# jalberse/shimmer

Hardware: AMD Instinct MI355X
Metric: Mray/s (primary+secondary) at 1024^2 256spp Ganesha; 1/2/4/8-GPU scaling (higher is better)
Workload: dtype f32

## Files before the change

### include/shimmer_hip.h

```cpp
#ifndef SHIMMER_HIP_H
#define SHIMMER_HIP_H

#include <stdint.h>

#ifdef __cplusplus
extern "C" {
#endif

#define SHM_ABI_VERSION 10

#if defined(__GNUC__)
#define SHM_API __attribute__((visibility("default")))
#else
#define SHM_API
#endif

typedef enum ShmError {
    SHM_OK = 0,
    SHM_ERR_INVALID_ARGUMENT = -1,
    SHM_ERR_UNSUPPORTED = -2,
    SHM_ERR_DEVICE = -3,
    SHM_ERR_NO_DEVICE = -4,
    SHM_ERR_OUT_OF_MEMORY = -5,
    SHM_ERR_INTERNAL = -6
// ... 358 lines not shown
    double ms_gather;
    uint64_t gather_bytes;
} ShmStats;

typedef struct ShmRay {
    float o[3];
    float d[3];
    float t_max;
    float pad;
} ShmRay;

typedef struct ShmHit {
    int32_t prim;
    float t;
    float b0, b1, b2;
    float phi;
    uint32_t instance;
    uint32_t pad;
} ShmHit;

typedef struct ShmScene ShmScene;

SHM_API int shm_scene_create(const ShmSceneDesc* desc, int device, ShmScene** out);
SHM_API void shm_scene_destroy(ShmScene* scene);

SHM_API int shm_scene_shading_records(ShmScene* scene, uint64_t* n_records_out, double* build_ms_out);

SHM_API int shm_film_clear(ShmScene* scene);
SHM_API int shm_render_wave(ShmScene* scene, const ShmRenderParams* params, const ShmTile* tiles, uint32_t n_tiles,
                    int32_t sample_begin, int32_t sample_end, ShmStats* stats);
SHM_API int shm_film_read(ShmScene* scene, ShmFilmPixel* film_out);
SHM_API int shm_film_device_ptr(ShmScene* scene, void** ptr_out, uint64_t* bytes_out);

SHM_API int shm_render_device(ShmScene* scene, const ShmRenderParams* params, const ShmTile* tiles, uint32_t n_tiles,
                              ShmStats* stats);
SHM_API int shm_render(ShmScene* scene, const ShmRenderParams* params, const ShmTile* tiles, uint32_t n_tiles,
               ShmFilmPixel* film, ShmStats* stats);

SHM_API int shm_trace_closest(ShmScene* scene, const ShmRay* rays, uint32_t n, ShmHit* hits_out, ShmStats* stats);
SHM_API int shm_trace_any(ShmScene* scene, const ShmRay* rays, uint32_t n, uint8_t* occluded_out, ShmStats* stats);
SHM_API int shm_trace_closest_device(ShmScene* scene, const void* rays_dev, uint32_t n, void* hits_dev, int repeat,
                             ShmStats* stats);
SHM_API int shm_trace_any_device(ShmScene* scene, const void* rays_dev, uint32_t n, void* occluded_dev, int repeat,
                         ShmStats* stats);


SHM_API int shm_shard_tiles(uint32_t n_tiles, uint32_t tiles_per_row, int32_t rank, int32_t world, int32_t rows_per_block,
                            uint32_t* idx_out, uint32_t* n_out);

#define SHM_DIST_ID_BYTES 128
SHM_API int shm_dist_unique_id(uint8_t id_out[SHM_DIST_ID_BYTES]);
SHM_API int shm_dist_init(ShmScene* scene, int32_t rank, int32_t world, const uint8_t id[SHM_DIST_ID_BYTES]);
SHM_API int shm_dist_finalize(ShmScene* scene);
SHM_API int shm_render_sharded(ShmScene* scene, const ShmRenderParams* params, ShmStats* stats);
enum { SHM_REDUCE_SUM = 0, SHM_REDUCE_MAX = 1, SHM_REDUCE_MIN = 2 };
SHM_API int shm_dist_barrier(ShmScene* scene);
SHM_API int shm_dist_allreduce_f64(ShmScene* scene, double* values , uint32_t n , int32_t op );
SHM_API int shm_dist_allgather_f64(ShmScene* scene, const double* mine, uint32_t n, double* all_out );
typedef struct ShmDistInfo {
    int32_t rank, world;
    int32_t rccl_ranks;
    int32_t rccl_device;
    int32_t rccl_version;
    int32_t hip_runtime_version;
    int32_t rows_per_block;
    uint32_t n_my_tiles;
    char librccl_path[256];
    char libamdhip_path[256];
} ShmDistInfo;
SHM_API int shm_dist_info(ShmScene* scene, ShmDistInfo* out);
SHM_API int shm_device_synchronize(int32_t device);
SHM_API int shm_dist_selftest(ShmScene* scene);

SHM_API int shm_render_multi(const ShmSceneDesc* desc, const int32_t* devices, int32_t n_devices, const ShmRenderParams* params,
                             ShmFilmPixel* film_out, ShmStats* stats_per_device);

SHM_API const char* shm_last_error(void);
SHM_API int shm_device_count(void);


SHM_API int shm_bvh_build(const float* prim_bounds, uint32_t n, int split_method, ShmBvhNode* nodes_out,
                  uint32_t* n_nodes_out, uint32_t* prim_order_out);
SHM_API int shm_bounds3_probe(const float a[6], const float b[6], const float p[3], float out[16]);
SHM_API int shm_tile_bounds(const int32_t pixel_bounds[4], int32_t tile_w, int32_t tile_h, ShmTile* tiles_out,
                    uint32_t* n_out);
SHM_API int shm_camera_perspective(const float world_from_camera[16], float fov_deg, const int32_t full_resolution[2],
                           float lens_radius, float focal_distance, ShmCamera* out,
                           float render_from_world_out[16]);
SHM_API int shm_camera_orthographic(const float world_from_camera[16], const int32_t full_resolution[2], float lens_radius,
                            float focal_distance, ShmCamera* out, float render_from_world_out[16]);
enum { SHM_RENDER_SPACE_CAMERA_WORLD = 0, SHM_RENDER_SPACE_CAMERA = 1, SHM_RENDER_SPACE_WORLD = 2 };
typedef struct ShmCameraParams {
    uint32_t kind;
    uint32_t render_space;
    float world_from_camera[16];
    float fov_deg;
    int32_t full_resolution[2];
    float lens_radius, focal_distance;
    float frame_aspect_ratio;
    uint32_t has_screen_window;
    float screen_window[4];
} ShmCameraParams;
SHM_API int shm_camera_create(const ShmCameraParams* params, ShmCamera* out, float render_from_world_out[16]);
SHM_API int shm_camera_spherical(const float world_from_camera[16], uint32_t mapping, const int32_t full_resolution[2], uint32_t render_space, ShmCamera* out,
                                 float render_from_world_out[16]);
SHM_API int shm_integrator_render(const char* name, const ShmSceneDesc* scene, int device, int32_t max_depth, int regularize,
                          int sample_lights, int sample_bsdf, int32_t samples_per_pixel, int32_t seed, int disable_pixel_jitter,
                          int disable_wavelength_jitter, ShmFilmPixel* film_out, ShmStats* stats_out, int32_t* n_waves_out);
SHM_API int shm_film_get_image(const ShmFilmPixel* film, uint64_t n_pixels, const float output_rgb_from_sensor_rgb[9], int write_fp16,
                       float* rgb_out);
SHM_API int shm_write_pfm(const char* path, const float* rgb, int32_t width, int32_t height);
typedef struct ShmPlyMesh {
    uint32_t n_vertices, n_tri_indices, n_quad_indices, n_face_indices;
    float* p;
    float* n;
    float* uv;
    int32_t* tri_indices;
    int32_t* quad_indices;
    int32_t* face_indices;
} ShmPlyMesh;
SHM_API int shm_ply_read(const char* filename, ShmPlyMesh* out);
SHM_API void shm_ply_free(ShmPlyMesh* mesh);

typedef struct ShmPbrtScene {
    ShmSceneDesc desc;
    ShmRenderParams params;
    char integrator[32];
    char output_filename[256];
    void* owner;
    float output_rgb_from_sensor_rgb[9];
} ShmPbrtScene;
SHM_API int shm_scene_load_pbrt(const char* path, ShmPbrtScene** out);
SHM_API int shm_scene_parse_pbrt(const char* text, const char* base_dir, ShmPbrtScene** out);
SHM_API void shm_pbrt_free(ShmPbrtScene* scene);
SHM_API int shm_pbrt_tokenize(const char* text, char* out, uint64_t capacity, uint32_t* n_tokens);
SHM_API int shm_pbrt_parse_params(const char* text, char* out_json, uint64_t capacity);
SHM_API int shm_blackbody_dense(float temperature_kelvin, float out471[471]);
SHM_API int shm_look_at(const float eye[3], const float look[3], const float up[3], float world_from_camera_out[16]);
typedef struct ShmLoadedImage {
    uint32_t n_levels, n_channels, file_channels, has_color_space;
    uint64_t n_texel_floats;
    ShmImageLevel* levels;
    float* texels;
} ShmLoadedImage;
SHM_API int shm_image_load_png(const char* path, const char* encoding, uint32_t wrap , int build_pyramid, ShmLoadedImage* out);
SHM_API void shm_image_free(ShmLoadedImage* image);

#ifdef __cplusplus
}
#endif
#endif
```

### shimmer_amd/abi.py

```python
import ctypes as C
import os
from pathlib import Path

ROOT = Path(__file__).resolve().parent
LIB_PATH = ROOT / "csrc" / "libshimmer_hip.so"

SHM_ABI_VERSION = 10
SHM_OK = 0
SHM_DIST_ID_BYTES = 128
SHM_SHAPE_TRIANGLE, SHM_SHAPE_SPHERE, SHM_SHAPE_BILINEAR_PATCH, SHM_SHAPE_INSTANCE = 0, 1, 2, 3
SHM_SPECTRUM_CONSTANT, SHM_SPECTRUM_DENSE, SHM_SPECTRUM_PIECEWISE_LINEAR = 0, 1, 2
SHM_SPECTRUM_RGB_ALBEDO, SHM_SPECTRUM_RGB_UNBOUNDED, SHM_SPECTRUM_RGB_ILLUMINANT = 3, 4, 5
SHM_MATERIAL_DIFFUSE, SHM_MATERIAL_CONDUCTOR, SHM_MATERIAL_DIELECTRIC, SHM_MATERIAL_THIN_DIELECTRIC = 0, 1, 2, 3
SHM_MATERIAL_COATED_DIFFUSE, SHM_MATERIAL_COATED_CONDUCTOR, SHM_MATERIAL_MIX = 4, 5, 6
SHM_MATERIAL_DIFFUSE_TRANSMISSION = 8
SHM_LIGHT_POINT, SHM_LIGHT_DIFFUSE_AREA, SHM_LIGHT_UNIFORM_INFINITE, SHM_LIGHT_IMAGE_INFINITE = 0, 1, 2, 3
SHM_LIGHT_DISTANT, SHM_LIGHT_SPOT = 4, 5
SHM_SPECTRUM_IMAGE_TEXTURE, SHM_SPECTRUM_TEXTURE_NODE = 6, 7
SHM_SPECTEX_LEAF, SHM_SPECTEX_SCALED, SHM_SPECTEX_MIX, SHM_SPECTEX_DIRECTION_MIX = 0, 1, 2, 3
SHM_TEXMAP_UV, SHM_TEXMAP_SPHERICAL, SHM_TEXMAP_CYLINDRICAL, SHM_TEXMAP_PLANAR = 0, 1, 2, 3
SHM_TEXMAP_POINT3D = 4
SHM_TEXFILTER_POINT, SHM_TEXFILTER_BILINEAR, SHM_TEXFILTER_TRILINEAR, SHM_TEXFILTER_EWA = 0, 1, 2, 3
SHM_FILTER_BOX, SHM_FILTER_GAUSSIAN, SHM_FILTER_MITCHELL, SHM_FILTER_SINC, SHM_FILTER_TRIANGLE = 0, 1, 2, 3, 4
SHM_WRAP_BLACK, SHM_WRAP_CLAMP, SHM_WRAP_REPEAT, SHM_WRAP_OCTAHEDRAL_SPHERE = 0, 1, 2, 3
# ... 144 lines not shown

class ShmRenderParams(C.Structure):
    _fields_ = [("seed", C.c_uint64), ("samples_per_pixel", C.c_int32), ("max_depth", C.c_int32), ("regularize", C.c_uint8),
                ("disable_pixel_jitter", C.c_uint8), ("disable_wavelength_jitter", C.c_uint8), ("force_diffuse", C.c_uint8),
                ("integrator", C.c_uint8), ("sample_lights", C.c_uint8), ("sample_bsdf", C.c_uint8), ("disable_texture_filtering", C.c_uint8),
                ("disable_reference_quirks", C.c_uint8), ("sampler", C.c_uint8), ("sampler_randomization", C.c_uint8), ("pad", C.c_uint8 * 5)]


class ShmTile(C.Structure):
    _fields_ = [("x0", C.c_int32), ("y0", C.c_int32), ("x1", C.c_int32), ("y1", C.c_int32)]


class ShmFilmPixel(C.Structure):
    _fields_ = [("rgb_sum", C.c_double * 3), ("weight_sum", C.c_double)]


class ShmStats(C.Structure):
    _fields_ = [("paths", C.c_uint64), ("rays_closest", C.c_uint64), ("rays_any", C.c_uint64), ("nodes_closest", C.c_uint64),
                ("tris_closest", C.c_uint64), ("nodes_any", C.c_uint64), ("tris_any", C.c_uint64), ("ms_total", C.c_double),
                ("ms_trace_closest", C.c_double), ("ms_trace_any", C.c_double), ("ms_shade", C.c_double),
                ("launches_closest", C.c_uint32), ("launches_any", C.c_uint32), ("ms_gather", C.c_double), ("gather_bytes", C.c_uint64)]

    def as_dict(self):
        return {name: getattr(self, name) for name, _ in self._fields_}


class ShmRay(C.Structure):
    _fields_ = [("o", C.c_float * 3), ("d", C.c_float * 3), ("t_max", C.c_float), ("pad", C.c_float)]


class ShmHit(C.Structure):
    _fields_ = [("prim", C.c_int32), ("t", C.c_float), ("b0", C.c_float), ("b1", C.c_float), ("b2", C.c_float),
                ("phi", C.c_float), ("instance", C.c_uint32), ("pad", C.c_uint32)]


assert C.sizeof(ShmMaterial) == 64 + 4 * 32 + 48 and C.sizeof(ShmFloatTexture) == 48 and C.sizeof(ShmBvhNode) == 32 and C.sizeof(ShmRay) == 32 and C.sizeof(ShmHit) == 32 and C.sizeof(ShmFilmPixel) == 32

class ShmPbrtScene(C.Structure):
    _fields_ = [("desc", ShmSceneDesc), ("params", ShmRenderParams), ("integrator", C.c_char * 32), ("output_filename", C.c_char * 256), ("owner", C.c_void_p),
                ("output_rgb_from_sensor_rgb", C.c_float * 9)]


class ShmCameraParams(C.Structure):
    _fields_ = [("kind", C.c_uint32), ("render_space", C.c_uint32), ("world_from_camera", C.c_float * 16), ("fov_deg", C.c_float),
                ("full_resolution", C.c_int32 * 2), ("lens_radius", C.c_float), ("focal_distance", C.c_float), ("frame_aspect_ratio", C.c_float),
                ("has_screen_window", C.c_uint32), ("screen_window", C.c_float * 4)]


class ShmLoadedImage(C.Structure):
    _fields_ = [("n_levels", C.c_uint32), ("n_channels", C.c_uint32), ("file_channels", C.c_uint32), ("has_color_space", C.c_uint32),
                ("n_texel_floats", C.c_uint64), ("levels", C.POINTER(ShmImageLevel)), ("texels", c_float_p)]


class ShmDistInfo(C.Structure):
    _fields_ = [("rank", C.c_int32), ("world", C.c_int32), ("rccl_ranks", C.c_int32), ("rccl_device", C.c_int32), ("rccl_version", C.c_int32),
                ("hip_runtime_version", C.c_int32), ("rows_per_block", C.c_int32), ("n_my_tiles", C.c_uint32), ("librccl_path", C.c_char * 256),
                ("libamdhip_path", C.c_char * 256)]

    def as_dict(self):
        return {n: (getattr(self, n).decode() if n.endswith("_path") else getattr(self, n)) for n, _ in self._fields_}


SHM_REDUCE_SUM, SHM_REDUCE_MAX, SHM_REDUCE_MIN = 0, 1, 2

EXPORTS = {
    "shm_scene_create": (C.c_int, [C.POINTER(ShmSceneDesc), C.c_int, C.POINTER(C.c_void_p)]),
    "shm_scene_destroy": (None, [C.c_void_p]),
    "shm_film_clear": (C.c_int, [C.c_void_p]),
    "shm_scene_shading_records": (C.c_int, [C.c_void_p, C.POINTER(C.c_uint64), C.POINTER(C.c_double)]),
    "shm_render_wave": (C.c_int, [C.c_void_p, C.POINTER(ShmRenderParams), C.POINTER(ShmTile), C.c_uint32, C.c_int32, C.c_int32,
                                  C.POINTER(ShmStats)]),
    "shm_film_read": (C.c_int, [C.c_void_p, C.c_void_p]),
    "shm_film_device_ptr": (C.c_int, [C.c_void_p, C.POINTER(C.c_void_p), C.POINTER(C.c_uint64)]),
    "shm_render_device": (C.c_int, [C.c_void_p, C.POINTER(ShmRenderParams), C.POINTER(ShmTile), C.c_uint32, C.POINTER(ShmStats)]),
    "shm_render": (C.c_int, [C.c_void_p, C.POINTER(ShmRenderParams), C.POINTER(ShmTile), C.c_uint32, C.c_void_p, C.POINTER(ShmStats)]),
    "shm_trace_closest": (C.c_int, [C.c_void_p, C.c_void_p, C.c_uint32, C.c_void_p, C.POINTER(ShmStats)]),
    "shm_trace_any": (C.c_int, [C.c_void_p, C.c_void_p, C.c_uint32, C.c_void_p, C.POINTER(ShmStats)]),
    "shm_trace_closest_device": (C.c_int, [C.c_void_p, C.c_void_p, C.c_uint32, C.c_void_p, C.c_int, C.POINTER(ShmStats)]),
    "shm_trace_any_device": (C.c_int, [C.c_void_p, C.c_void_p, C.c_uint32, C.c_void_p, C.c_int, C.POINTER(ShmStats)]),
    "shm_last_error": (C.c_char_p, []),
    "shm_device_count": (C.c_int, []),
    "shm_bvh_build": (C.c_int, [c_float_p, C.c_uint32, C.c_int, C.POINTER(ShmBvhNode), c_u32_p, c_u32_p]),
    "shm_bounds3_probe": (C.c_int, [c_float_p, c_float_p, c_float_p, c_float_p]),
    "shm_tile_bounds": (C.c_int, [C.POINTER(C.c_int32), C.c_int32, C.c_int32, C.POINTER(ShmTile), c_u32_p]),
    "shm_camera_perspective": (C.c_int, [c_float_p, C.c_float, C.POINTER(C.c_int32), C.c_float, C.c_float, C.POINTER(ShmCamera), c_float_p]),
    "shm_integrator_render": (C.c_int, [C.c_char_p, C.POINTER(ShmSceneDesc), C.c_int, C.c_int32, C.c_int, C.c_int, C.c_int, C.c_int32, C.c_int32, C.c_int, C.c_int,
                                        C.c_void_p, C.POINTER(ShmStats), C.POINTER(C.c_int32)]),
    "shm_camera_orthographic": (C.c_int, [c_float_p, C.POINTER(C.c_int32), C.c_float, C.c_float, C.POINTER(ShmCamera), c_float_p]),
    "shm_film_get_image": (C.c_int, [C.c_void_p, C.c_uint64, c_float_p, C.c_int, c_float_p]),
    "shm_write_pfm": (C.c_int, [C.c_char_p, c_float_p, C.c_int32, C.c_int32]),
    "shm_ply_read": (C.c_int, [C.c_char_p, C.c_void_p]),
    "shm_ply_free": (None, [C.c_void_p]),
    "shm_shard_tiles": (C.c_int, [C.c_uint32, C.c_uint32, C.c_int32, C.c_int32, C.c_int32, c_u32_p, c_u32_p]),
    "shm_dist_unique_id": (C.c_int, [C.c_void_p]),
    "shm_dist_init": (C.c_int, [C.c_void_p, C.c_int32, C.c_int32, C.c_void_p]),
    "shm_dist_finalize": (C.c_int, [C.c_void_p]),
    "shm_render_sharded": (C.c_int, [C.c_void_p, C.POINTER(ShmRenderParams), C.POINTER(ShmStats)]),
    "shm_dist_selftest": (C.c_int, [C.c_void_p]),
    "shm_dist_barrier": (C.c_int, [C.c_void_p]),
    "shm_dist_allreduce_f64": (C.c_int, [C.c_void_p, C.POINTER(C.c_double), C.c_uint32, C.c_int32]),
    "shm_dist_allgather_f64": (C.c_int, [C.c_void_p, C.POINTER(C.c_double), C.c_uint32, C.POINTER(C.c_double)]),
    "shm_dist_info": (C.c_int, [C.c_void_p, C.POINTER(ShmDistInfo)]),
    "shm_device_synchronize": (C.c_int, [C.c_int32]),
    "shm_scene_load_pbrt": (C.c_int, [C.c_char_p, C.POINTER(C.POINTER(ShmPbrtScene))]),
    "shm_scene_parse_pbrt": (C.c_int, [C.c_char_p, C.c_char_p, C.POINTER(C.POINTER(ShmPbrtScene))]),
    "shm_pbrt_free": (None, [C.POINTER(ShmPbrtScene)]),
    "shm_pbrt_tokenize": (C.c_int, [C.c_char_p, C.c_char_p, C.c_uint64, c_u32_p]),
    "shm_pbrt_parse_params": (C.c_int, [C.c_char_p, C.c_char_p, C.c_uint64]),
    "shm_blackbody_dense": (C.c_int, [C.c_float, c_float_p]),
    "shm_look_at": (C.c_int, [c_float_p, c_float_p, c_float_p, c_float_p]),
    "shm_image_load_png": (C.c_int, [C.c_char_p, C.c_char_p, C.c_uint32, C.c_int, C.POINTER(ShmLoadedImage)]),
    "shm_image_free": (None, [C.POINTER(ShmLoadedImage)]),
    "shm_camera_create": (C.c_int, [C.POINTER(ShmCameraParams), C.POINTER(ShmCamera), c_float_p]),
    "shm_camera_spherical": (C.c_int, [c_float_p, C.c_uint32, C.POINTER(C.c_int32), C.c_uint32, C.POINTER(ShmCamera), c_float_p]),
    "shm_render_multi": (C.c_int, [C.POINTER(ShmSceneDesc), C.POINTER(C.c_int32), C.c_int32, C.POINTER(ShmRenderParams), C.c_void_p, C.POINTER(ShmStats)]),
}

_lib = None


class ShimmerHipError(RuntimeError):
    pass


def load_library(path=None):
    global _lib
    if _lib is not None and path is None:
        return _lib
    if path is None and os.environ.get("SHM_LIB"):
        path = os.environ["SHM_LIB"]
    p = Path(path) if path else LIB_PATH
    if not p.exists():
        raise ShimmerHipError(f"{p} not found: run `python -c 'import __graft_entry__ as g; g.build()'` "
                              "(hipcc --offload-arch=gfx950). There is no CPU fallback for the render path.")
    lib = C.CDLL(str(p), mode=getattr(os, "RTLD_NOW", 2))
    host_only = os.environ.get("SHM_HOST_ONLY") == "1"
    for name, (res, args) in EXPORTS.items():
        if host_only and not hasattr(lib, name):
            continue
        fn = getattr(lib, name)
        fn.restype = res
        fn.argtypes = args
    if path is None:
        _lib = lib
    return lib


PROBE_LIB_PATH = LIB_PATH.parent / "libshimmer_hip_probe.so"
_probe = None


def load_probe_library():
    global _probe
    if _probe is None:
        if not PROBE_LIB_PATH.exists():
            raise ShimmerHipError(f"{PROBE_LIB_PATH} not found: run `python -c 'import __graft_entry__ as g; g.build()'`")
        lib = C.CDLL(str(PROBE_LIB_PATH), mode=getattr(os, "RTLD_NOW", 2))
        lib.shm_debug_eval_leaf.restype = C.c_int
        lib.shm_debug_eval_leaf.argtypes = [C.c_int, C.c_int, c_u32_p, C.c_uint32, c_u32_p, C.c_uint32, C.POINTER(C.c_int)]
        lib.shm_probe_last_error.restype = C.c_char_p
        _probe = lib
    return _probe


def check(lib, rc, what):
    if rc != SHM_OK:
# ... 3 lines not shown
```

### shimmer_amd/csrc/host/flatten.h

```cpp
#pragma once
#include <stdio.h>
#include <stdlib.h>

#include <algorithm>
#include <cmath>
#include <string>
#include <utility>
#include <vector>

#include "../shm/filter.h"
#include "../shm/scene.h"

static_assert(sizeof(ShmMaterial) == 240 && sizeof(ShmFloatTexture) == 48 && sizeof(ShmSpectrumTexture) == 64 && sizeof(ShmSpectrum) == 32 && sizeof(ShmBvhNode) == 32 && sizeof(ShmPrimitive) == 16,
              "POD layouts of include/shimmer_hip.h (mirrored by shimmer_amd/abi.py)");
namespace shm_host {

struct FlatScene {
    std::vector<ShmBvhNode> nodes;
    std::vector<shm::PrimRec> prim_recs;
    std::vector<ShmPrimitive> primitives;
    std::vector<uint32_t> mesh_flags;
    std::vector<uint32_t> vi;
    std::vector<float> vn, vs, vuv;
    std::vector<ShmSphere> spheres;
    std::vector<shm::PatchExtra> patches;
    std::vector<uint32_t> patch_vi;
    std::vector<float> patch_vn, patch_vuv;
    std::vector<ShmMaterial> materials;
    std::vector<ShmLight> lights;
    std::vector<shm::PrimRec> light_prim_recs;
    bool has_diffuse_transmission = false;
    bool has_directed_lights = false;
    std::vector<uint32_t> infinite_lights;
    std::vector<float> spectrum_data;
    std::vector<float> sensor_r, sensor_g, sensor_b;
    ShmCamera camera;
    ShmFilm film;
    uint32_t max_leaf_depth = 0;
    float scene_radius = 0.0f;
    uint64_t n_quadric_patch_prims = 0;
    bool has_spheres = false;
    bool has_layered = false;
    bool has_rough_dielectric = false;
    bool has_class[4] = {false, false, false, false};
    bool diffuse_only = true;
    std::vector<ShmImageTexture> image_textures;
    std::vector<ShmImageLevel> image_levels;
    std::vector<float> texel_data;
    std::vector<float> rgb2spec_scale, rgb2spec_data, cs_illuminant, ewa_lut;
    uint32_t rgb2spec_res = 0;
    bool has_textures = false;
    bool has_material_textures = false, has_image_light = false;
    double area_plain_diffuse = 0.0, area_total = 0.0;
    uint64_t n_plain_diffuse_prims = 0;
    std::vector<ShmInstance> instances;
    bool has_instances = false;
    std::vector<ShmFloatTexture> float_textures;
    std::vector<shm::FloatTexRange> ftex_ranges;
    std::vector<shm::FloatTexOp> ftex_ops;
    std::vector<ShmSpectrumTexture> spectrum_textures;
    std::vector<shm::FloatTexRange> stex_ranges;
    std::vector<shm::FloatTexOp> stex_ops;
    std::vector<shm::ImageLightRec> image_lights;
    std::vector<float> dist_data;

    shm::SceneView view() const {
        shm::SceneView v;
        v.quirks_off = 0;
        v.zsobol = 0;
        v.call_copy = nullptr;
        v.inst_roots = nullptr;
        v.tri_shade = nullptr;
        v.nodes = nodes.data();
        v.n_nodes = (uint32_t)nodes.size();
        v.prim_recs = prim_recs.data();
        v.primitives = primitives.data();
        v.n_primitives = (uint32_t)primitives.size();
        v.mesh_flags = mesh_flags.data();
        v.vi = vi.data();
        v.vn = vn.data();
        v.vs = vs.data();
        v.vuv = vuv.data();
        v.spheres = spheres.data();
        v.patches = patches.data();
        v.patch_vi = patch_vi.data();
        v.patch_vn = patch_vn.data();
        v.patch_vuv = patch_vuv.data();
        v.materials = materials.data();
        v.lights = lights.data();
        v.n_lights = (uint32_t)lights.size();
        v.light_prim_recs = light_prim_recs.empty() ? nullptr : light_prim_recs.data();
        v.infinite_lights = infinite_lights.data();
        v.n_infinite_lights = (uint32_t)infinite_lights.size();
        v.spectrum_data = spectrum_data.data();
        v.scene_radius = scene_radius;
        v.camera = camera;
        for (int i = 0; i < 4; ++i) v.pixel_bounds[i] = film.pixel_bounds[i];
        v.filter_radius[0] = film.filter_radius[0];
        v.filter_radius[1] = film.filter_radius[1];
        v.filter_kind = film.filter;
        v.imaging_ratio = film.imaging_ratio;
        v.max_component_value = film.max_component_value;
        v.sensor_r_bar = sensor_r.data();
        v.sensor_g_bar = sensor_g.data();
        v.sensor_b_bar = sensor_b.data();
        v.image_textures = image_textures.data();
        v.image_levels = image_levels.data();
        v.texel_data = texel_data.data();
        v.rgb2spec_res = rgb2spec_res;
        v.rgb2spec_scale = rgb2spec_scale.data();
        v.rgb2spec_data = rgb2spec_data.data();
        v.cs_illuminant = cs_illuminant.data();
        v.ewa_lut = ewa_lut.data();
        v.instances = instances.data();
        v.float_textures = float_textures.data();
        v.ftex_ranges = ftex_ranges.data();
        v.ftex_ops = ftex_ops.data();
        v.spectrum_textures = spectrum_textures.data();
        v.stex_ranges = stex_ranges.data();
        v.stex_ops = stex_ops.data();
        v.image_lights = image_lights.data();
        v.dist_data = dist_data.data();
        return v;
    }
};

inline bool check_spectrum(const ShmSpectrum& s, uint32_t n_floats, std::string& err, uint32_t n_textures = 0, bool* is_texture = nullptr) {
    if (s.kind == SHM_SPECTRUM_TEXTURE_NODE) {
        if (!is_texture) { err = "a spectrum texture is not valid in this slot"; return false; }
        *is_texture = true;
        return true;
    }
    if (s.kind == SHM_SPECTRUM_IMAGE_TEXTURE) {
        if (s.offset >= n_textures) { err = n_textures ? "image texture index out of range" : "an image texture is not valid in this slot"; return false; }
        if (is_texture) *is_texture = true;
        return true;
    }
    if (s.kind == SHM_SPECTRUM_CONSTANT || s.kind == SHM_SPECTRUM_RGB_ALBEDO || s.kind == SHM_SPECTRUM_RGB_UNBOUNDED) return true;
    if (s.kind == SHM_SPECTRUM_DENSE || s.kind == SHM_SPECTRUM_RGB_ILLUMINANT) {
        if ((uint64_t)s.offset + s.n > n_floats) { err = "dense spectrum out of range"; return false; }
        return true;
    }
    if (s.kind == SHM_SPECTRUM_PIECEWISE_LINEAR) {
        if (s.n < 2 || (uint64_t)s.offset + 2ull * s.n > n_floats) { err = "piecewise spectrum out of range"; return false; }
        return true;
    }
    err = "unknown spectrum kind";
    return false;
}

inline float build_pc1d(const float* f, size_t n, std::vector<float>& pool, size_t func_off, size_t cdf_off) {
    for (size_t i = 0; i < n; ++i) pool[func_off + i] = f[i] < 0.0f ? -f[i] : f[i];
    pool[cdf_off] = 0.0f;
    for (size_t i = 1; i <= n; ++i) pool[cdf_off + i] = pool[cdf_off + i - 1] + pool[func_off + i - 1] * (1.0f - 0.0f) / (float)n;
    const float func_int = pool[cdf_off + n];
// ... 485 lines not shown
    out.light_prim_recs.assign(out.lights.size(), shm::PrimRec{});
    for (uint32_t i = 0; i < out.lights.size(); ++i)
        if (out.lights[i].kind == SHM_LIGHT_DIFFUSE_AREA) out.light_prim_recs[i] = out.prim_recs[out.lights[i].primitive];
    for (uint32_t i = 0; i < out.lights.size(); ++i) {
        if (out.lights[i].kind != SHM_LIGHT_SPOT) continue;
        const ShmSpotLight& sp = d->spot_lights[out.lights[i].primitive];
        shm::PrimRec& r = out.light_prim_recs[i];
        for (int k = 0; k < 3; ++k) { r.p0[k] = sp.light_from_render[k]; r.p1[k] = sp.light_from_render[4 + k]; r.p2[k] = sp.light_from_render[8 + k]; }
        r.mesh = shm::float_to_bits(sp.cos_falloff_start);
        r.tri = shm::float_to_bits(sp.cos_falloff_end);
    }

    if (d->n_instances) out.instances.assign(d->instances, d->instances + d->n_instances);
    {
        struct Item { uint32_t node, depth; bool inner; };
        std::vector<Item> st;
        st.push_back({0u, 0u, false});
        uint64_t visited = 0;
        const uint64_t visit_cap = (uint64_t)d->n_nodes * (1ull + d->n_instances);
        while (!st.empty()) {
            auto [i, depth, inner] = st.back();
            st.pop_back();
            if (i >= d->n_nodes) { err = "BVH child index out of range"; return SHM_ERR_INVALID_ARGUMENT; }
            if (++visited > visit_cap) { err = "BVH is not a tree"; return SHM_ERR_INVALID_ARGUMENT; }
            const ShmBvhNode& n = d->nodes[i];
            if (n.n_prims > 0) {
                if ((uint64_t)n.offset + n.n_prims > d->n_primitives) { err = "BVH leaf range out of bounds"; return SHM_ERR_INVALID_ARGUMENT; }
                if (depth > out.max_leaf_depth) out.max_leaf_depth = depth;
                for (uint32_t k = 0; k < n.n_prims; ++k) {
                    const ShmPrimitive& pr = out.primitives[n.offset + k];
                    if (pr.shape_kind != SHM_SHAPE_INSTANCE) {
                        if (inner && pr.area_light >= 0) { err = "an instanced primitive cannot carry an area light"; return SHM_ERR_UNSUPPORTED; }
                        continue;
                    }
                    if (inner) { err = "an instanced primitive cannot itself be an instance"; return SHM_ERR_UNSUPPORTED; }
                    if (n.n_prims != 1) { err = "an instance must be alone in its BVH leaf"; return SHM_ERR_UNSUPPORTED; }
                    const ShmInstance& in = out.instances[pr.shape_index];
                    if (in.root_node == 0 || in.root_node >= d->n_nodes) { err = "instance root node out of range"; return SHM_ERR_INVALID_ARGUMENT; }
                    st.push_back({in.root_node, depth + 2, true});
                }
            } else {
                if (n.axis > 2) { err = "BVH axis out of range"; return SHM_ERR_INVALID_ARGUMENT; }
                if (n.offset <= i) { err = "BVH second child must follow its parent"; return SHM_ERR_INVALID_ARGUMENT; }
                st.push_back({n.offset, depth + 1, inner});
                st.push_back({i + 1, depth + 1, inner});
            }
        }
    }
    if (getenv("SHM_DEBUG")) fprintf(stderr, "[shm] flatten: %u nodes, %u prims, max leaf depth %u\n", d->n_nodes, d->n_primitives, out.max_leaf_depth);
    if (out.max_leaf_depth >= 64) { err = "BVH deeper than the reference's 64-entry traversal stack"; return SHM_ERR_UNSUPPORTED; }
    for (ShmMaterial& m : out.materials) {
        if (m.kind == SHM_MATERIAL_DIFFUSE_TRANSMISSION) {
            ShmSpectrum zero;
            memset(&zero, 0, sizeof(zero));
            zero.kind = SHM_SPECTRUM_CONSTANT;
            m.c = m.d = zero;
            m.conductor_from_reflectance = 0;
            for (int k = 1; k < 8; ++k) m.float_tex[k] = 0u;
        }
        const bool tex_a = m.a.kind == SHM_SPECTRUM_IMAGE_TEXTURE || m.a.kind == SHM_SPECTRUM_TEXTURE_NODE;
        bool any_float_tex = false;
        for (int k = 0; k < 8; ++k) any_float_tex = any_float_tex || m.float_tex[k] != 0u;
        m.pad[0] = (m.kind == SHM_MATERIAL_DIFFUSE && !tex_a && !any_float_tex && m.normal_map == 0u) ? 1u : 0u;
    }
    for (const shm::PrimRec& pr : out.prim_recs) {
        const bool plain = pr.material < out.materials.size() && (out.materials[pr.material].pad[0] & 1u);
        if (plain) out.n_plain_diffuse_prims += 1u;
        double area = 0.0;
        if (pr.kind_index & shm::PRIM_SPHERE_BIT) { const double r = d->spheres[pr.kind_index & shm::PRIM_INDEX_MASK].radius; area = 4.0 * 3.14159265358979 * r * r; }
        else if (pr.kind_index & shm::PRIM_PATCH_BIT) area = out.patches[pr.kind_index & shm::PRIM_INDEX_MASK].area;
        else if (!(pr.kind_index & shm::PRIM_INSTANCE_BIT)) {
            const double ax = (double)pr.p1[0] - pr.p0[0], ay = (double)pr.p1[1] - pr.p0[1], az = (double)pr.p1[2] - pr.p0[2];
            const double bx = (double)pr.p2[0] - pr.p0[0], by = (double)pr.p2[1] - pr.p0[1], bz = (double)pr.p2[2] - pr.p0[2];
            const double cx = ay * bz - az * by, cy = az * bx - ax * bz, cz = ax * by - ay * bx;
            area = 0.5 * std::sqrt(cx * cx + cy * cy + cz * cz);
        }
        if (area == area && area < 1e300) { out.area_total += area; if (plain) out.area_plain_diffuse += area; }
    }
    out.has_material_textures = out.has_textures;
    out.has_textures = out.has_material_textures || out.has_image_light;
    return SHM_OK;
}

}
```

### shimmer_amd/csrc/host/host_mirror.cpp

```cpp
#include <stdio.h>
#include <string.h>

#include <algorithm>
#include <atomic>
#include <cmath>
#include <new>
#include <stdexcept>
#include <string>
#include <thread>
#include <vector>

#include "../../../include/shimmer_hip.h"
#include "../shm/path.h"

extern "C" __attribute__((visibility("hidden"))) void shm_set_last_error(const char* msg);

namespace {

struct B3 {
    float mn[3], mx[3];
};
inline B3 b3_default() {
    B3 b;
    for (int i = 0; i < 3; ++i) { b.mn[i] = 3.40282346638528859812e+38f; b.mx[i] = -3.40282346638528859812e+38f; }
    return b;
}
inline float fmin_rs(float a, float b) { return (b != b) ? a : ((a != a) ? b : (a < b ? a : b)); }
inline float fmax_rs(float a, float b) { return (b != b) ? a : ((a != a) ? b : (a > b ? a : b)); }
inline B3 b3_union(const B3& a, const B3& b) {
    B3 r;
    for (int i = 0; i < 3; ++i) { r.mn[i] = fmin_rs(a.mn[i], b.mn[i]); r.mx[i] = fmax_rs(a.mx[i], b.mx[i]); }
    return r;
}
inline B3 b3_union_point(const B3& a, const float p[3]) {
    B3 r;
    for (int i = 0; i < 3; ++i) { r.mn[i] = fmin_rs(a.mn[i], p[i]); r.mx[i] = fmax_rs(a.mx[i], p[i]); }
    return r;
}
inline float b3_surface_area(const B3& b) {
    float dx = b.mx[0] - b.mn[0], dy = b.mx[1] - b.mn[1], dz = b.mx[2] - b.mn[2];
    return 2.0f * (dx * dy + dx * dz + dy * dz);
}
inline int b3_max_dimension(const B3& b) {
    float dx = b.mx[0] - b.mn[0], dy = b.mx[1] - b.mn[1], dz = b.mx[2] - b.mn[2];
    if (dx > dy && dx > dz) return 0;
    return (dy > dz) ? 1 : 2;
}

struct BvhPrimitive {
    uint32_t primitive_index;
    B3 bounds;
    float centroid(int dim) const {
        return 0.5f * bounds.mn[dim] + bounds.mx[dim] * 0.5f;
    }
};

struct BuildNode {
    B3 bounds;
    int left = -1, right = -1;
    uint8_t split_axis = 0;
    uint32_t first_prim_offset = 0;
    uint32_t n_primitives = 0;
};

struct BuildTask {
    size_t begin, end;
    int top_index;
    std::vector<BuildNode> nodes;
};
constexpr uint32_t TASK_PLACEHOLDER = 0xffffffffu;

struct Builder {
    BvhPrimitive* prims;
    std::vector<BuildNode> build_nodes;
    uint32_t* ordered;
    int split_method;
    std::vector<BuildTask>* tasks = nullptr;
    size_t grain = 0;

    template <typename Pred>
    static size_t partition(BvhPrimitive* a, size_t n, Pred pred) {
        size_t split_index = 0;
        size_t front = 0, back = n;
        while (front < back) {
            if (!pred(a[front])) {
                bool swapped = false;
                while (back > front + 1) {
                    --back;
                    if (pred(a[back])) {
                        std::swap(a[front], a[back]);
                        swapped = true;
                        break;
                    }
                }
                if (!swapped) break;
            }
// ... 65 lines not shown
            return mid;
        };
        if (split_method == 0) {
            float pmid = (cb.mn[dim] + cb.mx[dim]) / 2.0f;
            split_index = partition(prims + begin, n, [dim, pmid](const BvhPrimitive& p) { return p.centroid(dim) < pmid; });
            if (split_index == 0 || split_index == n) split_index = median_split();
        } else {
            split_index = median_split();
        }
        int left = build(begin, begin + split_index);
        int right = build(begin + split_index, end);
        BuildNode& node = build_nodes[node_idx];
        node.bounds = b3_union(build_nodes[left].bounds, build_nodes[right].bounds);
        node.left = left;
        node.right = right;
        node.split_axis = (uint8_t)dim;
        return node_idx;
    }
};

thread_local std::string g_host_err;

struct M4 {
    double m[4][4];
};
M4 m4_identity() {
    M4 r;
    for (int i = 0; i < 4; ++i) for (int j = 0; j < 4; ++j) r.m[i][j] = (i == j) ? 1.0 : 0.0;
    return r;
}
M4 m4_mul(const M4& a, const M4& b) {
    M4 r;
    for (int i = 0; i < 4; ++i)
        for (int j = 0; j < 4; ++j) {
            double s = 0;
            for (int k = 0; k < 4; ++k) s += a.m[i][k] * b.m[k][j];
            r.m[i][j] = s;
        }
    return r;
}
bool m4_inverse(const M4& a, M4& out) {
    double aug[4][8];
    for (int i = 0; i < 4; ++i)
        for (int j = 0; j < 4; ++j) { aug[i][j] = a.m[i][j]; aug[i][j + 4] = (i == j) ? 1.0 : 0.0; }
    for (int c = 0; c < 4; ++c) {
        int piv = c;
        for (int r = c + 1; r < 4; ++r) if (std::fabs(aug[r][c]) > std::fabs(aug[piv][c])) piv = r;
        if (aug[piv][c] == 0.0) return false;
        if (piv != c) for (int j = 0; j < 8; ++j) std::swap(aug[c][j], aug[piv][j]);
        double inv = 1.0 / aug[c][c];
        for (int j = 0; j < 8; ++j) aug[c][j] *= inv;
        for (int r = 0; r < 4; ++r) {
            if (r == c) continue;
            double f = aug[r][c];
            if (f != 0.0) for (int j = 0; j < 8; ++j) aug[r][j] -= f * aug[c][j];
        }
    }
    for (int i = 0; i < 4; ++i) for (int j = 0; j < 4; ++j) out.m[i][j] = aug[i][j + 4];
    return true;
}
M4 m4_scale(double x, double y, double z) { M4 r = m4_identity(); r.m[0][0] = x; r.m[1][1] = y; r.m[2][2] = z; return r; }
M4 m4_translate(double x, double y, double z) { M4 r = m4_identity(); r.m[0][3] = x; r.m[1][3] = y; r.m[2][3] = z; return r; }
void m4_to_f32(const M4& a, float* out) { for (int i = 0; i < 4; ++i) for (int j = 0; j < 4; ++j) out[i * 4 + j] = (float)a.m[i][j]; }
void m4_point(const M4& a, const double p[3], double out[3]) {
    double r[4];
    for (int i = 0; i < 4; ++i) r[i] = a.m[i][0] * p[0] + a.m[i][1] * p[1] + a.m[i][2] * p[2] + a.m[i][3];
    for (int i = 0; i < 3; ++i) out[i] = (r[3] == 1.0) ? r[i] : r[i] / r[3];
}

}

extern "C" {

int shm_bounds3_probe(const float a[6], const float b[6], const float p[3], float out[16]) {
    if (!a || !b || !p || !out) return SHM_ERR_INVALID_ARGUMENT;
    B3 ba, bb;
    for (int k = 0; k < 3; ++k) { ba.mn[k] = a[k]; ba.mx[k] = a[3 + k]; bb.mn[k] = b[k]; bb.mx[k] = b[3 + k]; }
    const B3 u = b3_union(ba, bb), up = b3_union_point(ba, p);
    for (int k = 0; k < 3; ++k) { out[k] = u.mn[k]; out[3 + k] = u.mx[k]; out[6 + k] = up.mn[k]; out[9 + k] = up.mx[k]; }
    out[12] = b3_surface_area(ba);
    out[13] = (ba.mx[0] - ba.mn[0]) * (ba.mx[1] - ba.mn[1]) * (ba.mx[2] - ba.mn[2]);
    out[14] = (float)b3_max_dimension(ba);
    out[15] = 0.0f;
    return SHM_OK;
}

int shm_bvh_build(const float* prim_bounds, uint32_t n, int split_method, ShmBvhNode* nodes_out,
                  uint32_t* n_nodes_out, uint32_t* prim_order_out) {
    if (!prim_bounds || n == 0 || !nodes_out || !n_nodes_out || !prim_order_out || split_method < 0 || split_method > 1)
        return SHM_ERR_INVALID_ARGUMENT;
    std::vector<BvhPrimitive> prims(n);
    for (uint32_t i = 0; i < n; ++i) {
        prims[i].primitive_index = i;
        for (int k = 0; k < 3; ++k) {
            prims[i].bounds.mn[k] = prim_bounds[6ull * i + k];
            prims[i].bounds.mx[k] = prim_bounds[6ull * i + 3 + k];
            if (prim_bounds[6ull * i + k] != prim_bounds[6ull * i + k]) return SHM_ERR_INVALID_ARGUMENT;
        }
    }
    unsigned n_threads = std::min(std::max(std::thread::hardware_concurrency(), 1u), 64u);
    if (const char* e = getenv("SHM_BVH_THREADS")) { const int v = atoi(e); if (v >= 1 && v <= 1024) n_threads = (unsigned)v; }
    if (n < 65536u) n_threads = 1;
    std::vector<BuildTask> tasks;
    Builder b;
    b.prims = prims.data();
    b.build_nodes.reserve(n_threads > 1 ? 1024 : 2ull * n);
    b.ordered = prim_order_out;
    b.split_method = split_method;
    if (n_threads > 1) { b.tasks = &tasks; b.grain = n / 64u; b.fold_threads = std::min(n_threads, 16u); }
    b.build(0, n);
    if (!tasks.empty()) {
        std::atomic<size_t> next{0};
        auto worker = [&]() {
            for (size_t t = next.fetch_add(1); t < tasks.size(); t = next.fetch_add(1)) {
                Builder sub;
                sub.prims = prims.data();
                sub.ordered = prim_order_out;
                sub.split_method = split_method;
                sub.build_nodes.reserve(2 * (tasks[t].end - tasks[t].begin));
                sub.build(tasks[t].begin, tasks[t].end);
                tasks[t].nodes.swap(sub.build_nodes);
            }
        };
        std::vector<std::thread> pool;
        try {
            for (unsigned t = 1; t < std::min<size_t>(n_threads, tasks.size()); ++t) pool.emplace_back(worker);
        } catch (...) {}
        worker();
        for (std::thread& t : pool) t.join();
        auto bounds_of = [&](int i) -> const B3& { const BuildNode& c = b.build_nodes[i]; return c.n_primitives == TASK_PLACEHOLDER ? tasks[c.first_prim_offset].nodes[0].bounds : c.bounds; };
        for (size_t i = b.build_nodes.size(); i-- > 0;) {
            BuildNode& node = b.build_nodes[i];
            if (node.n_primitives == 0) node.bounds = b3_union(bounds_of(node.left), bounds_of(node.right));
        }
    }
    std::vector<uint32_t> final_index(b.build_nodes.size());
    uint64_t total64 = 0;
    for (size_t i = 0; i < b.build_nodes.size(); ++i) {
        final_index[i] = (uint32_t)total64;
        total64 += b.build_nodes[i].n_primitives == TASK_PLACEHOLDER ? tasks[b.build_nodes[i].first_prim_offset].nodes.size() : 1u;
    }
    if (total64 > 0xffffffffull) return SHM_ERR_UNSUPPORTED;
    const uint32_t total = (uint32_t)total64;
    std::atomic<int> rc_emit{SHM_OK};
    std::atomic<uint64_t> n_in_leaves{0};
    auto emit = [&](const BuildNode& bn, uint32_t base, ShmBvhNode& ln, uint64_t& leaf_prims) {
        memset(&ln, 0, sizeof(ln));
        for (int k = 0; k < 3; ++k) { ln.bmin[k] = bn.bounds.mn[k]; ln.bmax[k] = bn.bounds.mx[k]; }
        if (bn.n_primitives > 0) {
            if (bn.n_primitives >= 65536) rc_emit = SHM_ERR_UNSUPPORTED;
            ln.offset = bn.first_prim_offset;
            ln.n_prims = (uint16_t)bn.n_primitives;
            ln.axis = 0;
            leaf_prims += bn.n_primitives;
        } else {
            ln.offset = base;
            ln.n_prims = 0;
            ln.axis = bn.split_axis;
        }
    };
    {
        uint64_t leaf_prims = 0;
        for (size_t i = 0; i < b.build_nodes.size(); ++i) {
            const BuildNode& bn = b.build_nodes[i];
            if (bn.n_primitives == TASK_PLACEHOLDER) continue;
            emit(bn, bn.n_primitives == 0 ? final_index[bn.right] : 0u, nodes_out[final_index[i]], leaf_prims);
// ... 407 lines not shown
```

### shimmer_amd/csrc/render.hip

```cpp
#include <chrono>
#include "wavefront.h"
#include "host/integrator.hpp"

std::string& shm_err() {
    thread_local std::string e;
    return e;
}
#define g_err shm_err()

namespace {

__global__ void k_expand_tiles(const ShmTile* tiles, const uint32_t* tile_offset, uint32_t n_tiles, uint32_t* pixels) {
    uint32_t t = blockIdx.x * blockDim.x + threadIdx.x;
    if (t >= n_tiles) return;
    ShmTile tl = tiles[t];
    uint32_t k = tile_offset[t];
    for (int x = tl.x0; x < tl.x1; ++x)
        for (int y = tl.y0; y < tl.y1; ++y) pixels[k++] = (uint32_t)x | ((uint32_t)y << 16);
}

#include "k_generate.inl"

__global__ void __launch_bounds__(256) k_build_tri_shade(SceneView sv, PrimRec* prim_recs, TriShadeRec* recs, uint32_t n_prims, uint32_t* n_built, uint32_t plain_only) {
    const uint32_t i = blockIdx.x * blockDim.x + threadIdx.x;
// ... 148 lines not shown
};
struct FilterKernels {
    FilteredGenerateKernel generate[2][2];
    WeightedFilmKernel film;
};
template <bool ZS>
constexpr FilterKernels filter_cells[N_FLT - 1] = {
    {{{k_generate_filtered<false, false, ZS, FILTER_CLASS_TRIANGLE>, k_generate_filtered<false, true, ZS, FILTER_CLASS_TRIANGLE>}, {k_generate_filtered<true, false, ZS, FILTER_CLASS_TRIANGLE>, nullptr}}, nullptr},
    {{{k_generate_filtered<false, false, ZS, FILTER_CLASS_TABULATED>, k_generate_filtered<false, true, ZS, FILTER_CLASS_TABULATED>}, {k_generate_filtered<true, false, ZS, FILTER_CLASS_TABULATED>, nullptr}},
     k_film_weighted<FILM_WEIGHT_CONSTANT>},
    {{{k_generate_filtered<false, false, ZS, FILTER_CLASS_TABULATED>, k_generate_filtered<false, true, ZS, FILTER_CLASS_TABULATED>}, {k_generate_filtered<true, false, ZS, FILTER_CLASS_TABULATED>, nullptr}},
     k_film_weighted<FILM_WEIGHT_PER_SAMPLE>},
};
static ShadeKernels select_kernels(const RenderPlan& p) {
    const ShadeKernels(&cells)[N_GEO][N_IMG] = p.dl ? (p.zs ? shade_cells<true, true> : shade_cells<false, true>) : (p.zs ? shade_cells<true, false> : shade_cells<false, false>);
    ShadeKernels k = cells[p.geo][p.img];
    k.lean = cells[p.geo][p.img_lean].lean;
    k.lean_diverted = cells[p.geo][p.img_lean].lean_diverted;
    k.generate[0] = cells[p.geo][p.img_generate].generate[0];
    k.generate[1] = cells[p.geo][p.img_generate].generate[1];
    k.generate_filtered[0] = k.generate_filtered[1] = nullptr;
    k.film_weighted = nullptr;
    if (p.flt != FLT_BOX) {
        const FilterKernels& fk = (p.zs ? filter_cells<true> : filter_cells<false>)[p.flt - 1];
        k.generate_filtered[0] = fk.generate[p.img_generate == IMG_TEX ? 1 : 0][0];
        k.generate_filtered[1] = fk.generate[p.img_generate == IMG_TEX ? 1 : 0][1];
        k.film_weighted = fk.film;
    }
    if (p.layered_onepass) k.scatter[CLASS_LAYERED] = k.scatter_layered_onepass;
    if (p.spherical) {
        const SphericalGenerateCells& sc = wf_generate_spherical(p.zs);
        const int tex = p.img_generate == IMG_TEX ? 1 : 0;
        for (int lean = 0; lean < 2; ++lean) {
            k.generate[lean] = sc.generate[tex][lean];
            k.generate_filtered[lean] = p.flt != FLT_BOX ? sc.generate_filtered[p.flt == FLT_TRIANGLE ? 0 : 1][tex][lean] : nullptr;
        }
    }
    return k;
}
template <bool ZS, bool DL>
constexpr bool cells_match_plan() {
    for (int g = 0; g < N_GEO; ++g)
        for (int i = 0; i < N_IMG; ++i) {
            const ShadeKernels& c = shade_cells<ZS, DL>[g][i];
            if ((c.lean != nullptr) != HAS_LEAN_KERNELS[i] || (c.lean_diverted != nullptr) != HAS_LEAN_KERNELS[i] || (c.generate[1] != nullptr) != HAS_LEAN_KERNELS[i]) return false;
        }
    return true;
}
static_assert(cells_match_plan<true, true>() && cells_match_plan<false, true>() && cells_match_plan<true, false>() && cells_match_plan<false, false>(), "shade_cells vs HAS_LEAN_KERNELS");
static bool kernels_complete(const ShadeKernels& k, const ScenePlan& sp, const RenderPlan& p) {
    bool ok = p.flt != FLT_BOX ? k.generate_filtered[p.lean_first ? 1 : 0] != nullptr : k.generate[p.lean_first ? 1 : 0] != nullptr;
    if (p.route == ROUTE_LEAN) ok = ok && k.lean;
    if (p.route == ROUTE_SIMPLE) ok = ok && k.simple;
    if (p.route == ROUTE_RANDOM_WALK) ok = ok && k.randomwalk;
    if (p.route == ROUTE_STAGED && p.fused_from != NEVER) ok = ok && k.fused_all;
    if (p.staged_bounce(0)) {
        ok = ok && k.vertex && (!p.drain_lean || k.lean_diverted);
        for (int c = 0; c < N_BXDF_CLASSES; ++c) ok = ok && (!sp.f.has_class[c] || k.scatter[c]);
    }
    return ok;
}
static uint64_t workspace_cap(const ShmScene* s, bool need_staged) {
    const uint64_t BYTES_PER_PATH = ws_bytes_per_path(s->plan, ws_staged_layout(s->plan, need_staged, s->ws_staged));
    uint64_t cap = max_batch_paths();
    size_t free_b = 0, total_b = 0;
    if (hipMemGetInfo(&free_b, &total_b) == hipSuccess) {
        uint64_t avail = (uint64_t)free_b + (uint64_t)s->capacity * BYTES_PER_PATH;
        uint64_t by_mem = (uint64_t)((double)avail * 0.8) / BYTES_PER_PATH;
        if (by_mem < cap) cap = by_mem;
    }
    return std::max<uint64_t>(cap, 4096);
}

}
LdsTables wf_lds_tables(const ShmScene* s, uint32_t budget) {
    LdsTables t = {};
    const shm_host::FlatScene& f = s->flat;
    auto pad16 = [](size_t b) { return (size_t)((b + 15u) & ~(size_t)15u); };
    const size_t want[N_LDS_TABLES] = {
        pad16(f.mesh_flags.size() * sizeof(uint32_t)), pad16(f.lights.size() * sizeof(ShmLight)), pad16(f.light_prim_recs.size() * sizeof(shm::PrimRec)), pad16(f.materials.size() * sizeof(ShmMaterial)), pad16(f.spectrum_data.size() * sizeof(float)),
        pad16(f.rgb2spec_scale.size() * sizeof(float)),
        pad16(f.image_textures.size() * sizeof(ShmImageTexture)), pad16(f.image_levels.size() * sizeof(ShmImageLevel)), pad16(f.float_textures.size() * sizeof(ShmFloatTexture)),
        pad16(f.ftex_ranges.size() * sizeof(shm::FloatTexRange)), pad16(f.ftex_ops.size() * sizeof(shm::FloatTexOp)), pad16(f.spectrum_textures.size() * sizeof(ShmSpectrumTexture)),
        pad16(f.stex_ranges.size() * sizeof(shm::FloatTexRange)), pad16(f.stex_ops.size() * sizeof(shm::FloatTexOp)), pad16(f.ewa_lut.size() * sizeof(float))};
    size_t left = budget;
    for (int k = 0; k < N_LDS_TABLES; ++k)
        if (want[k] && want[k] <= left) { t.bytes[k] = (uint32_t)want[k]; left -= want[k]; }
    return t;
}
namespace {
int ensure_workspace(ShmScene* s, uint64_t needed_paths, bool need_staged) {
    uint64_t max_cap = workspace_cap(s, need_staged);
    uint64_t want = std::min<uint64_t>(std::max<uint64_t>(needed_paths, 4096), max_cap);
    need_staged = ws_staged_layout(s->plan, need_staged, s->ws_staged);
    if (s->ws_staged || !need_staged) {
        if (s->capacity >= want) return SHM_OK;
        if (needed_paths > max_cap && s->capacity * 10ull >= max_cap * 9ull) return SHM_OK;
    }
    if (want > max_cap / 8) want = max_cap;
    want = (want + 4095ull) & ~4095ull;
    if (want > 0xfffff000ull) want = 0xfffff000ull;
    want = std::max<uint64_t>(want, s->capacity);
    if (want >= (1ull << 30)) { g_err = "internal: path workspace of 2^30 paths or more"; return SHM_ERR_INTERNAL; }
    for (void* p : s->ws_allocs) hipFree(p);
    s->ws_allocs.clear();
    s->capacity = 0;
    s->ws_staged = false;
    const uint32_t cap = (uint32_t)want;
    auto ws_alloc = [&](size_t bytes, void** out) -> int {
        void* d = nullptr;
        if (hipMalloc(&d, bytes) != hipSuccess) { g_err = "hipMalloc of the path workspace failed"; return SHM_ERR_OUT_OF_MEMORY; }
        s->ws_allocs.push_back(d);
        *out = d;
        return SHM_OK;
    };
    const ScenePlan& p = s->plan;
    const bool staged = need_staged;
    int rc;
#define WS_ALLOC(id, field, bytes, when)                                                        \
    static_assert(sizeof(*s->field) == bytes, "SHM_WS_ARRAYS: bytes per path of " #id);         \
    s->field = nullptr;                                                                         \
    if ((when) && (rc = ws_alloc((size_t)cap * bytes, (void**)&s->field)) != SHM_OK) return rc;
    SHM_WS_ARRAYS(WS_ALLOC)
#undef WS_ALLOC
    s->pa.has_layered = p.f.has_class[CLASS_LAYERED] ? 1u : 0u;
    s->ws_staged = staged;
    s->capacity = cap;
    DBG("workspace: %u paths", cap);
    return SHM_OK;
}
struct BatchHitState {
    ShmScene* s;
    ShmHit* const base;
    BatchHitState(ShmScene* sc, const RenderPlan& p) : s(sc), base(sc->pa.hit) {
        s->pa.hit16 = p.hit16 ? 1u : 0u;
        s->pa.hit2 = p.hit_split ? reinterpret_cast<const float4*>(base) + s->capacity : nullptr;
    }
    void keep_previous(int bounce) {
        float4* const h16 = reinterpret_cast<float4*>(base);
        s->pa.hit = reinterpret_cast<ShmHit*>(h16 + (size_t)(bounce & 1) * s->capacity);
        s->pa.hit_prev = h16 + (size_t)((bounce + 1) & 1) * s->capacity;
    }
    ~BatchHitState() { s->pa.hit = base; s->pa.hit_prev = nullptr; s->pa.hit16 = 0u; s->pa.hit2 = nullptr; }
};

int upload_scene(ShmScene* s) {
    const shm_host::FlatScene& f = s->flat;
    SceneView v = f.view();
    shm_host::BvhPairs bvh;
    int rc = shm_host::bvh_pairs(f, bvh, g_err);
    if (rc != SHM_OK) return rc;
#define UP(vec, field) if ((rc = dev_upload(s, vec, &v.field)) != SHM_OK) return rc
    UP(bvh.nodes, nodes);
    if (!bvh.big_leaf_n.empty()) { const uint32_t* d = nullptr; if ((rc = dev_upload(s, bvh.big_leaf_n, &d)) != SHM_OK) return rc; s->d_big_leaf_n = const_cast<uint32_t*>(d); }
    UP(f.prim_recs, prim_recs); UP(f.primitives, primitives); UP(f.mesh_flags, mesh_flags); UP(f.vi, vi); UP(f.vn, vn); UP(f.vs, vs); UP(f.vuv, vuv);
    UP(f.spheres, spheres); UP(f.patches, patches); UP(f.patch_vi, patch_vi); UP(f.patch_vn, patch_vn); UP(f.patch_vuv, patch_vuv);
    UP(f.materials, materials); UP(f.lights, lights);
    v.light_prim_recs = nullptr;
    if (!f.light_prim_recs.empty()) UP(f.light_prim_recs, light_prim_recs);
    UP(f.infinite_lights, infinite_lights); UP(f.spectrum_data, spectrum_data); UP(f.sensor_r, sensor_r_bar); UP(f.sensor_g, sensor_g_bar); UP(f.sensor_b, sensor_b_bar);
    UP(f.image_textures, image_textures); UP(f.image_levels, image_levels); UP(f.texel_data, texel_data); UP(f.rgb2spec_scale, rgb2spec_scale);
    UP(f.rgb2spec_data, rgb2spec_data); UP(f.cs_illuminant, cs_illuminant); UP(f.ewa_lut, ewa_lut);
    UP(bvh.instances, instances); UP(bvh.inst_roots, inst_roots);
    UP(f.float_textures, float_textures); UP(f.ftex_ranges, ftex_ranges); UP(f.ftex_ops, ftex_ops);
    UP(f.spectrum_textures, spectrum_textures); UP(f.stex_ranges, stex_ranges); UP(f.stex_ops, stex_ops);
    UP(f.image_lights, image_lights); UP(f.dist_data, dist_data);
#undef UP
    v.tri_shade = nullptr;
    s->dsv = v;
    size_t w = (size_t)(f.film.pixel_bounds[2] - f.film.pixel_bounds[0]);
    size_t h = (size_t)(f.film.pixel_bounds[3] - f.film.pixel_bounds[1]);
    s->n_film_pixels = w * h;
    if ((rc = dev_alloc<ShmFilmPixel>(s, s->n_film_pixels, &s->d_film)) != SHM_OK) return rc;
    if (hipMemset(s->d_film, 0, s->n_film_pixels * sizeof(ShmFilmPixel)) != hipSuccess) { g_err = "hipMemset film"; return SHM_ERR_DEVICE; }
    if ((rc = dev_alloc<QueueState>(s, 1, &s->d_qs)) != SHM_OK) return rc;
    if ((rc = dev_alloc<DeviceCounters>(s, 1, &s->d_counters)) != SHM_OK) return rc;
    uint32_t* heads = nullptr;
    if ((rc = dev_alloc<uint32_t>(s, N_RAY * TRACE_QUEUE_PARTS * TRACE_HEAD_STRIDE, &heads)) != SHM_OK) return rc;
    for (int ray = 0; ray < N_RAY; ++ray) s->trace[ray].d_heads = heads + ray * TRACE_QUEUE_PARTS * TRACE_HEAD_STRIDE;
    hipMemset(s->d_qs, 0, sizeof(QueueState));
    hipMemset(s->d_counters, 0, sizeof(DeviceCounters));
    return SHM_OK;
}
int build_tri_shade(ShmScene* s) {
    const shm_host::FlatScene& f = s->flat;
    TriShadeRec* recs = nullptr;
    uint32_t* d_n = nullptr;
    int rc;
    if ((rc = dev_alloc<TriShadeRec>(s, f.prim_recs.size(), &recs)) != SHM_OK) return rc;
    if ((rc = dev_alloc<uint32_t>(s, 1, &d_n)) != SHM_OK) return rc;
    const uint32_t n_prims = (uint32_t)f.prim_recs.size();
    const auto t0 = std::chrono::steady_clock::now();
    uint32_t n_built = 0;
    hipError_t err = hipMemset(d_n, 0, sizeof(uint32_t));
    if (err == hipSuccess) {
        hipLaunchKernelGGL(k_build_tri_shade, dim3((n_prims + 255u) / 256u), dim3(256), 0, 0, s->dsv, const_cast<PrimRec*>(s->dsv.prim_recs), recs, n_prims, d_n,
                           s->plan.tri_shade_plain_only ? 1u : 0u);
        err = hipGetLastError();
    }
    if (err == hipSuccess) err = hipDeviceSynchronize();
    if (err == hipSuccess) err = hipMemcpy(&n_built, d_n, sizeof(uint32_t), hipMemcpyDeviceToHost);
    if (err != hipSuccess) { g_err = std::string("k_build_tri_shade: ") + hipGetErrorString(err); return SHM_ERR_DEVICE; }
    s->n_tri_shade_records = n_built;
    s->tri_shade_build_ms = std::chrono::duration<double, std::milli>(std::chrono::steady_clock::now() - t0).count();
    DBG("scene: %u shading records of %u primitives built in %.3f ms (%.1f MB)", n_built, n_prims, s->tri_shade_build_ms, (double)n_prims * sizeof(TriShadeRec) / 1e6);
    s->dsv.tri_shade = recs;
    return SHM_OK;
}
}

extern "C" {

const char* shm_last_error(void) { return g_err.c_str(); }
__attribute__((visibility("hidden"))) void shm_set_last_error(const char* msg) { g_err = msg ? msg : ""; }

int shm_device_count(void) {
    int n = 0;
    if (hipGetDeviceCount(&n) != hipSuccess) return 0;
    return n;
}

void shm_scene_destroy(ShmScene* s) {
    if (!s) return;
    hipSetDevice(s->device);
    wf_trace_census();
    wf_layered_census();
    wf_dist_release(s);
    for (void* p : s->allocs) hipFree(p);
    for (void* p : s->ws_allocs) hipFree(p);
    if (s->d_rw) hipFree(s->d_rw);
    if (s->d_tiles) hipFree(s->d_tiles);
    if (s->d_tile_offset) hipFree(s->d_tile_offset);
    if (s->d_pixels) hipFree(s->d_pixels);
    for (hipEvent_t e : s->events) hipEventDestroy(e);
    if (s->stream2) hipStreamDestroy(s->stream2);
    for (hipStream_t st : s->stream_cls) if (st) hipStreamDestroy(st);
    if (s->stream) hipStreamDestroy(s->stream);
    delete s;
}

int shm_scene_create(const ShmSceneDesc* desc, int device, ShmScene** out) {
    if (!out) { g_err = "out is null"; return SHM_ERR_INVALID_ARGUMENT; }
// ... 480 lines not shown
```

### shimmer_amd/csrc/shm/patch.h

```cpp
#pragma once
#include "shapes.h"

namespace shm {

struct PatchData {
    V3 p00, p10, p01, p11;
    bool flip;
    bool is_rect;
    Float area;
    bool has_n, has_uv;
    V3 n00, n10, n01, n11;
    V2 uv00, uv10, uv01, uv11;
};
SHM_HD V2 lerp2(Float t, V2 a, V2 b) { return a * (1.0f - t) + b * t; }
SHM_HD V3 blp_interp_normal(const PatchData& pd, Float u, Float v);
struct BilinearIntersection {
    Float u, v, t;
};

SHM_HD V3 lerp3(Float t, V3 a, V3 b) { return a * (1.0f - t) + b * t; }

SHM_HD bool quadratic(Float a, Float b, Float c, Float& t0, Float& t1) {
    if (a == 0.0f) {
        if (b == 0.0f) return false;
// ... 112 lines not shown
SHM_HD SurfaceInteraction blp_interaction(const PatchData& pd, Float u, Float v, V3 wo) {
    V3 p = lerp3(u, lerp3(v, pd.p00, pd.p01), lerp3(v, pd.p10, pd.p11));
    V3 dpdu = lerp3(v, pd.p10, pd.p11) - lerp3(v, pd.p00, pd.p01);
    V3 dpdv = lerp3(u, pd.p01, pd.p11) - lerp3(u, pd.p00, pd.p10);
    V2 st = v2(u, v);
    Float duds = 1.0f, dudt = 0.0f, dvds = 0.0f, dvdt = 1.0f;
    if (pd.has_uv) {
        st = lerp2(u, lerp2(v, pd.uv00, pd.uv01), lerp2(v, pd.uv10, pd.uv11));
        V2 dstdu = lerp2(v, pd.uv10, pd.uv11) - lerp2(v, pd.uv00, pd.uv01);
        V2 dstdv = lerp2(u, pd.uv01, pd.uv11) - lerp2(u, pd.uv00, pd.uv10);
        duds = (abs(dstdu.x) < 1e-8f) ? 0.0f : 1.0f / dstdu.x;
        dvds = (abs(dstdv.x) < 1e-8f) ? 0.0f : 1.0f / dstdv.x;
        dudt = (abs(dstdu.y) < 1e-8f) ? 0.0f : 1.0f / dstdu.y;
        dvdt = (abs(dstdv.y) < 1e-8f) ? 0.0f : 1.0f / dstdv.y;
        V3 dpds = dpdu * duds + dpdv * dvds;
        V3 dpdt = dpdu * dudt + dpdv * dvdt;
        if (cross(dpds, dpdt) != v3s(0.0f)) {
            if (dot(cross(dpdu, dpdv), cross(dpds, dpdt)) < 0.0f) dpdt = -dpdt;
            dpdu = dpds;
            dpdv = dpdt;
        }
    }
    V3 d2pduu = v3s(0.0f), d2pdvv = v3s(0.0f);
    V3 d2pduv = (pd.p00 - pd.p01) + (pd.p11 - pd.p10);
    Float e1 = dot(dpdu, dpdu), f1 = dot(dpdu, dpdv), g1 = dot(dpdv, dpdv);
    V3 n = normalize(cross(dpdu, dpdv));
    Float e2 = dot(n, d2pduu), f2 = dot(n, d2pduv), g2 = dot(n, d2pdvv);
    Float egf2 = difference_of_products(e1, g1, f1, f1);
    Float inv_egf2 = (egf2 != 0.0f) ? 1.0f / egf2 : 0.0f;
    V3 dndu = (f1 * f2 - e2 * g1) * inv_egf2 * dpdu + (e2 * f1 - f2 * e1) * inv_egf2 * dpdv;
    V3 dndv = (g2 * f1 - f2 * g1) * inv_egf2 * dpdu + (f2 * f1 - g2 * e1) * inv_egf2 * dpdv;
    V3 dnds = dndu * duds + dndv * dvds;
    V3 dndt = dndu * dudt + dndv * dvdt;
    dndu = dnds;
    dndv = dndt;
    V3 p_abs_sum = abs3(pd.p00) + abs3(pd.p01) + abs3(pd.p10) + abs3(pd.p11);
    V3 p_error = gamma(6) * p_abs_sum;
    SurfaceInteraction isect = surface_interaction_new(p3i_from_value_and_error(p, p_error), st, wo, dpdu, dpdv, dndu, dndv, pd.flip);
    if (pd.has_n) {
        V3 ns = blp_interp_normal(pd, u, v);
        if (length_squared(ns) > 0.0f) {
            ns = normalize(ns);
            V3 dndu_s = lerp3(v, pd.n10, pd.n11) - lerp3(v, pd.n00, pd.n01);
            V3 dndv_s = lerp3(u, pd.n01, pd.n11) - lerp3(u, pd.n00, pd.n10);
            V3 dnds_s = dndu_s * duds + dndv_s * dvds;
            V3 dndt_s = dndu_s * dudt + dndv_s * dvdt;
            Rot3 r = rotate_from_to(isect.n, ns);
            set_shading_geometry(isect, ns, rot3_apply(r, dpdu), rot3_apply(r, dpdv), dnds_s, dndt_s, true);
        }
    }
    return isect;
}

SHM_HD Float cross2d(V2 a, V2 b) { return difference_of_products(a.x, b.y, a.y, b.x); }
SHM_HD V2 invert_bilinear(V2 p, V2 v0, V2 v1, V2 v2_, V2 v3_) {
    V2 a = v0, b = v1, c = v3_, d = v2_;
    V2 e = b - a, f = d - a, g = (a - b) + (c - d), h = p - a;
    Float k2 = cross2d(g, f);
    Float k1 = cross2d(e, f) + cross2d(h, g);
    Float k0 = cross2d(h, e);
    if (abs(k2) < 0.001f) {
        if (abs(e.x * k1 - g.x * k0) < 1e-5f) return v2((h.y * k1 + f.y * k0) / (e.y * k1 - g.y * k0), -k0 / k1);
        return v2((h.x * k1 + f.x * k0) / (e.x * k1 - g.x * k0), -k0 / k1);
    }
    Float r0, r1;
    if (!quadratic(k2, k1, k0, r0, r1)) return v2(0.0f, 0.0f);
    Float u = (h.x - f.x * r0) / (e.x + g.x * r0);
    if (u < 0.0f || u > 1.0f || r0 < 0.0f || r0 > 1.0f) return v2((h.x - f.x * r1) / (e.x + g.x * r1), r1);
    return v2(u, r0);
}

SHM_HD Float spherical_quad_area(V3 a, V3 b, V3 c, V3 d) {
    V3 axb = cross(a, b), bxc = cross(b, c), cxd = cross(c, d), dxa = cross(d, a);
    if (length_squared(axb) == 0.0f || length_squared(bxc) == 0.0f || length_squared(cxd) == 0.0f || length_squared(dxa) == 0.0f)
        return 0.0f;
    axb = normalize(axb); bxc = normalize(bxc); cxd = normalize(cxd); dxa = normalize(dxa);
    Float alpha = angle_between(dxa, -axb);
    Float beta = angle_between(axb, -bxc);
    Float gamma_ = angle_between(bxc, -cxd);
    Float delta = angle_between(cxd, -dxa);
    return abs(alpha + beta + gamma_ + delta - 2.0f * PI_F);
}

SHM_HD V3 sample_spherical_rectangle(V3 p_ref, V3 s, V3 ex, V3 ey, V2 u, Float& pdf) {
    Float exl = length(ex), eyl = length(ey);
    Frame r;
    r.x = ex / exl;
    r.y = ey / eyl;
    r.z = cross(r.x, r.y);
    V3 d_local = r.to_local(s - p_ref);
    Float z0 = d_local.z;
    if (z0 > 0.0f) {
        r.z = -r.z;
        z0 *= -1.0f;
    }
    Float x0 = d_local.x, y0 = d_local.y;
    Float x1 = x0 + exl, y1 = y0 + eyl;
    V3 v00 = v3(x0, y0, z0), v01 = v3(x0, y1, z0), v10 = v3(x1, y0, z0), v11 = v3(x1, y1, z0);
    V3 n0 = normalize(cross(v00, v10)), n1 = normalize(cross(v10, v11)), n2 = normalize(cross(v11, v01)), n3 = normalize(cross(v01, v00));
    Float g0 = angle_between(-n0, n1), g1 = angle_between(-n1, n2), g2 = angle_between(-n2, n3), g3 = angle_between(-n3, n0);
    Float solid_angle = g0 + g1 + g2 + g3 - 2.0f * PI_F;
    if (solid_angle <= 0.0f) {
        pdf = 0.0f;
        return s + u.x * ex + u.y * ey;
    }
    pdf = max(0.0f, 1.0f / solid_angle);
    if (solid_angle < 1e-3f) return s + u.x * ex + u.y * ey;
    Float b0 = n0.z, b1 = n2.z;
    Float au = u.x * (g0 + g1 - 2.0f * PI_F) + (u.x - 1.0f) * (g2 + g3);
    Float fu = (cos(au) * b0 - b1) / sin(au);
    Float cu = copysign(1.0f / sqrt(sqr(fu) + sqr(b0)), fu);
    cu = clamp(cu, -(1.0f - 1.1920929e-7f), 1.0f - 1.1920929e-7f);
    Float xu = -(cu * z0) / safe_sqrt(1.0f - sqr(cu));
    xu = clamp(xu, x0, x1);
    Float dd = sqrt(sqr(xu) + sqr(z0));
    Float h0 = y0 / sqrt(sqr(dd) + sqr(y0));
    Float h1 = y1 / sqrt(sqr(dd) + sqr(y1));
    Float hv = h0 + u.y * (h1 - h0);
    Float hvsq = sqr(hv);
    Float yv = (hvsq < 1.0f - 1e-6f) ? (hv * dd) / sqrt(1.0f - hvsq) : y1;
    return p_ref + r.from_local(v3(xu, yv, z0));
}

SHM_HD V2 invert_spherical_rectangle_sample(V3 p_ref, V3 s, V3 ex, V3 ey, V3 p_rect) {
    Float exl = length(ex), eyl = length(ey);
    Frame r;
    r.x = ex / exl;
    r.y = ey / eyl;
    r.z = cross(r.x, r.y);
    V3 d_local = r.to_local(s - p_ref);
    Float z0 = d_local.z;
    if (z0 > 0.0f) {
        r.z = -r.z;
        z0 *= -1.0f;
    }
    Float z0sq = sqr(z0);
    Float x0 = d_local.x, y0 = d_local.y;
    Float x1 = x0 + exl, y1 = y0 + eyl;
    Float y0sq = sqr(y0), y1sq = sqr(y1);
    V3 v00 = v3(x0, y0, z0), v01 = v3(x0, y1, z0), v10 = v3(x1, y0, z0), v11 = v3(x1, y1, z0);
    V3 n0 = normalize(cross(v00, v10)), n1 = normalize(cross(v10, v11)), n2 = normalize(cross(v11, v01)), n3 = normalize(cross(v01, v00));
    Float g0 = angle_between(-n0, n1), g1 = angle_between(-n1, n2), g2 = angle_between(-n2, n3), g3 = angle_between(-n3, n0);
    Float b0 = n0.z, b1 = n2.z;
    Float b0sq = sqr(b0);
    Float solid_angle = g0 + g1 + g2 + g3 - 2.0f * PI_F;
    if (solid_angle < 1e-3f) {
        V3 pq = p_rect - s;
        return v2(dot(pq, ex) / length_squared(ex), dot(pq, ey) / length_squared(ey));
    }
    V3 vl = r.to_local(p_rect - p_ref);
    Float xu = vl.x, yv = vl.y;
    xu = clamp(xu, x0, x1);
    if (xu == 0.0f) xu = 1e-10f;
    Float invcusq = 1.0f + z0sq / sqr(xu);
    Float fusq = invcusq - b0sq;
    Float fu = copysign(sqrt(fusq), xu);
    Float sq = safe_sqrt(difference_of_products(b0, b0, b1, b1) + fusq);
    Float au = atan2(-(b1 * fu) - copysign(b0 * sq, fu * b0), b0 * b1 - sq * abs(fu));
    if (au > 0.0f) au -= 2.0f * PI_F;
    if (fu == 0.0f) au = PI_F;
    Float u0 = (au + g2 + g3) / solid_angle;
    Float ddsq = sqr(xu) + z0sq;
    Float dd = sqrt(ddsq);
    Float h0 = y0 / sqrt(ddsq + y0sq);
    Float h1 = y1 / sqrt(ddsq + y1sq);
    Float yvsq = sqr(yv);
    Float u1a = (difference_of_products(h0, h0, h0, h1) - abs(h0 - h1) * sqrt(yvsq * (ddsq + yvsq)) / (ddsq + yvsq)) / sqr(h0 - h1);
    Float u1b = (difference_of_products(h0, h0, h0, h1) + abs(h0 - h1) * sqrt(yvsq * (ddsq + yvsq)) / (ddsq + yvsq)) / sqr(h0 - h1);
    Float hva = lerp(u1a, h0, h1), hvb = lerp(u1b, h0, h1);
    Float yza = (hva * dd) / sqrt(1.0f - sqr(hva)), yzb = (hvb * dd) / sqrt(1.0f - sqr(hvb));
    if (abs(yza - yv) < abs(yzb - yv)) return v2(clamp(u0, 0.0f, 1.0f), u1a);
    return v2(clamp(u0, 0.0f, 1.0f), u1b);
}

SHM_HD bool blp_sample(const PatchData& pd, V2 u, ShapeSample& out, bool strict = false) {
    V2 uv;
    Float pdf;
    if (pd.is_rect) {
        uv = u;
        pdf = 1.0f;
    } else {
        Float w[4] = {length(cross(pd.p10 - pd.p00, pd.p01 - pd.p00)), length(cross(pd.p10 - pd.p00, pd.p11 - pd.p10)),
                      length(cross(pd.p01 - pd.p00, pd.p11 - pd.p01)), length(cross(pd.p11 - pd.p10, pd.p11 - pd.p01))};
        uv = sample_bilinear(u, w);
        pdf = bilinear_pdf(uv, w);
    }
    V3 pu0 = strict ? lerp3(uv.y, pd.p00, pd.p01) : lerp3(uv.x, pd.p00, pd.p10);
    V3 pu1 = lerp3(uv.y, pd.p10, pd.p11);
    V3 p = lerp3(uv.x, pu0, pu1);
    V3 dpdu = pu1 - pu0;
    V3 dpdv = lerp3(uv.x, pd.p01, pd.p11) - lerp3(uv.x, pd.p00, pd.p10);
    if (length_squared(dpdu) == 0.0f || length_squared(dpdv) == 0.0f) return false;
    V3 n = normalize(cross(dpdu, dpdv));
    if (pd.has_n) n = face_forward(n, blp_interp_normal(pd, uv.x, uv.y));
    else if (pd.flip) n = -n;
    V3 p_abs_sum = abs3(pd.p00) + abs3(pd.p01) + abs3(pd.p10) + abs3(pd.p11);
    V3 p_error = gamma(6) * p_abs_sum;
    out.pi = p3i_from_value_and_error(p, p_error);
    out.n = n;
    out.pdf = pdf / length(cross(dpdu, dpdv));
    return true;
}
SHM_HD Float blp_pdf(const PatchData& pd, V2 uv, bool strict = false) {
    if (pd.has_uv) uv = invert_bilinear(uv, pd.uv00, pd.uv10, pd.uv01, pd.uv11);
    Float pdf = 1.0f;
    if (!pd.is_rect) {
        Float w[4] = {length(cross(pd.p10 - pd.p00, pd.p01 - pd.p00)), length(cross(pd.p10 - pd.p00, pd.p11 - pd.p10)),
                      length(cross(pd.p01 - pd.p00, pd.p11 - pd.p01)), length(cross(pd.p11 - pd.p10, pd.p11 - pd.p01))};
        pdf = bilinear_pdf(uv, w);
    }
    V3 pu0 = strict ? lerp3(uv.y, pd.p00, pd.p01) : lerp3(uv.y, pd.p00, pd.p10);
    V3 pu1 = lerp3(uv.y, pd.p10, pd.p11);
    V3 dpdu = pu1 - pu0;
    V3 dpdv = lerp3(uv.x, pd.p01, pd.p11) - lerp3(uv.x, pd.p00, pd.p10);
    return pdf / length(cross(dpdu, dpdv));
}

constexpr Float BLP_MIN_SPHERICAL_SAMPLE_AREA = 1e-4f;

SHM_HD bool blp_sample_with_context(const PatchData& pd, const ShapeSampleContext& ctx, V2 u, ShapeSample& out, bool strict = false) {
    V3 rp = ctx.p();
    V3 v00 = normalize(pd.p00 - rp), v10 = normalize(pd.p10 - rp), v01 = normalize(pd.p01 - rp), v11 = normalize(pd.p11 - rp);
    if (!pd.is_rect || spherical_quad_area(v00, v10, v11, v01) <= BLP_MIN_SPHERICAL_SAMPLE_AREA) {
        ShapeSample ss;
        if (!blp_sample(pd, u, ss, strict)) return false;
        V3 wi = ss.pi.mid() - rp;
        if (length_squared(wi) == 0.0f) return false;
        wi = normalize(wi);
        ss.pdf /= abs_dot(ss.n, -wi) / length_squared(rp - ss.pi.mid());
        if (is_inf(ss.pdf)) return false;
        out = ss;
        return true;
    }
    Float pdf = 1.0f;
    if (ctx.ns != v3s(0.0f)) {
        Float w[4] = {max(0.01f, dot(v00, ctx.ns)), max(0.01f, dot(v10, ctx.ns)), max(0.01f, dot(v01, ctx.ns)), max(0.01f, dot(v11, ctx.ns))};
        u = sample_bilinear(u, w);
        pdf = bilinear_pdf(u, w);
    }
    V3 eu = pd.p10 - pd.p00, ev = pd.p01 - pd.p00;
    Float quad_pdf = 0.0f;
    V3 p = sample_spherical_rectangle(rp, pd.p00, eu, ev, u, quad_pdf);
    pdf *= quad_pdf;
    V2 uv = v2(dot(p - pd.p00, eu) / distance_squared(pd.p10, pd.p00), dot(p - pd.p00, ev) / distance_squared(pd.p01, pd.p00));
    V3 n = normalize(cross(eu, ev));
    if (pd.has_n) n = face_forward(n, blp_interp_normal(pd, uv.x, uv.y));
    else if (pd.flip) n = -n;
    out.pi = p3i_exact(p);
    out.n = n;
    out.pdf = pdf;
    return true;
}

SHM_HD Float blp_pdf_with_context(const PatchData& pd, const ShapeSampleContext& ctx, V3 wi, bool strict = false) {
    V3 o = offset_ray_origin(ctx.pi, ctx.n, wi);
    BilinearIntersection bi;
    if (!blp_intersect(o, wi, infinity(), pd.p00, pd.p10, pd.p01, pd.p11, bi)) return 0.0f;
    SurfaceInteraction isect = blp_interaction(pd, bi.u, bi.v, -wi);
    V3 rp = ctx.p();
    V3 v00 = normalize(pd.p00 - rp), v10 = normalize(pd.p10 - rp), v01 = normalize(pd.p01 - rp), v11 = normalize(pd.p11 - rp);
    if (!pd.is_rect || spherical_quad_area(v00, v10, v11, v01) <= BLP_MIN_SPHERICAL_SAMPLE_AREA) {
        Float pdf = blp_pdf(pd, isect.uv, strict) * distance_squared(rp, isect.p()) / abs_dot(isect.n, -wi);
        return is_inf(pdf) ? 0.0f : pdf;
    }
    Float pdf = 1.0f / spherical_quad_area(v00, v10, v11, v01);
    if (ctx.ns != v3s(0.0f)) {
        Float w[4] = {max(0.01f, dot(v00, ctx.ns)), max(0.01f, dot(v10, ctx.ns)), max(0.01f, dot(v01, ctx.ns)), max(0.01f, dot(v11, ctx.ns))};
        V2 u = invert_spherical_rectangle_sample(rp, pd.p00, pd.p10 - pd.p00, pd.p01 - pd.p00, isect.p());
        return bilinear_pdf(u, w) * pdf;
    }
    return pdf;
}

}
```

### shimmer_amd/csrc/shm/path.h

```cpp
#pragma once
#include "bxdf.h"
#include "filter.h"
#include "scene.h"
#include "texture.h"

namespace shm {

struct LightSampleContext {
    P3i pi;
    V3 n, ns;
    SHM_HD V3 p() const { return pi.mid(); }
};
SHM_HD LightSampleContext light_ctx_from(const SurfaceInteraction& si) {
    LightSampleContext c;
    c.pi = si.pi; c.n = si.n; c.ns = si.shading.n;
    return c;
}
struct LightLiSample {
    Spec l;
    V3 wi;
    Float pdf;
    P3i p_light_pi;
    V3 p_light_n;
};

#ifndef SHM_DELTA_LIGHTS
#define SHM_DELTA_LIGHTS 1
#endif

SHM_HD bool light_is_delta(const ShmLight& l) {
    if (SHM_DELTA_LIGHTS && (l.kind == SHM_LIGHT_DISTANT || l.kind == SHM_LIGHT_SPOT)) return true;
    return l.kind == SHM_LIGHT_POINT;
}

SHM_HD Float smoothstep(Float x, Float a, Float b) {
    if (a == b) return x < a ? 0.0f : 1.0f;
    Float t = clamp((x - a) / (b - a), 0.0f, 1.0f);
    return t * t * (3.0f - 2.0f * t);
}
SHM_HD Float spot_cos_theta(const PrimRec& r, V3 w) {
    Float x = dot(ld3(r.p0), w);
    Float len2 = x * x;
    Float y = dot(ld3(r.p1), w);
    len2 = len2 + y * y;
    Float z = dot(ld3(r.p2), w);
    len2 = len2 + z * z;
    return z / sqrt(len2);
}

SHM_HD Spec area_light_l(const SceneView& sv, const ShmLight& light, V3 n, V3 w, const Wavelengths& lambda) {
    if (!light.two_sided && dot(n, w) < 0.0f) return spec_const(0.0f);
    return light.scale * spectrum_sample(light.spectrum, sv.spectrum_data, lambda);
}

template <bool TRI_ONLY = false, bool HAS_TEX = false>
SHM_HD bool light_sample_li(const SceneView& sv, const ShmLight& light, const LightSampleContext& ctx, V2 u,
                            const Wavelengths& lambda, LightLiSample& out, bool allow_incomplete_pdf = true) {
    if (HAS_TEX && light.kind == SHM_LIGHT_IMAGE_INFINITE) {
        const ImageLightRec& il = sv.image_lights[light.primitive];
        Float map_pdf;
        V2 uv = pc2d_sample(sv.dist_data, allow_incomplete_pdf ? il.compensated : il.distribution, (int)il.n, u, map_pdf);
        if (map_pdf == 0.0f) return false;
        V3 w_light = equal_area_square_to_sphere(uv);
        V3 wi = xf_vector(il.render_from_light, w_light);
        out.l = light.scale * image_light_le_uv(sv, il, uv, lambda);
        out.wi = wi;
        out.pdf = map_pdf / (4.0f * PI_F);
        out.p_light_pi = p3i_exact(ctx.p() + wi * (2.0f * sv.scene_radius));
        out.p_light_n = v3s(0.0f);
        return true;
    }
    if (light.kind == SHM_LIGHT_POINT) {
        V3 p = ld3(light.position);
        V3 wi = normalize(p - ctx.p());
        Spec li = light.scale * spectrum_sample(light.spectrum, sv.spectrum_data, lambda) / distance_squared(p, ctx.p());
        out.l = li; out.wi = wi; out.pdf = 1.0f;
        out.p_light_pi = p3i_exact(p);
        out.p_light_n = v3s(0.0f);
        return true;
    }
    if (SHM_DELTA_LIGHTS && light.kind == SHM_LIGHT_SPOT) {
        V3 p = ld3(light.position);
        V3 wi = normalize(p - ctx.p());
        Float d2 = distance_squared(p, ctx.p());
        Spec i = spectrum_sample(light.spectrum, sv.spectrum_data, lambda);
        const PrimRec& r = light_side_rec(sv, light);
        Float falloff = smoothstep(spot_cos_theta(r, -wi), bits_to_float(r.tri), bits_to_float(r.mesh));
        Spec li = falloff * light.scale * i / d2;
        if (is_zero(li)) return false;
        out.l = li; out.wi = wi; out.pdf = 1.0f;
        out.p_light_pi = p3i_exact(p);
        out.p_light_n = v3s(0.0f);
        return true;
    }
    if (SHM_DELTA_LIGHTS && light.kind == SHM_LIGHT_DISTANT) {
        V3 wi = ld3(light.position);
        out.l = light.scale * spectrum_sample(light.spectrum, sv.spectrum_data, lambda);
        out.wi = wi; out.pdf = 1.0f;
        out.p_light_pi = p3i_exact(ctx.p() + wi * (2.0f * sv.scene_radius));
        out.p_light_n = v3s(0.0f);
        return true;
    }
    if (light.kind == SHM_LIGHT_UNIFORM_INFINITE) {
        if (allow_incomplete_pdf) return false;
        V3 wi = sample_uniform_sphere(u);
        out.l = light.scale * spectrum_sample(light.spectrum, sv.spectrum_data, lambda);
        out.wi = wi;
        out.pdf = uniform_hemisphere_pdf(sv.quirks_off != 0);
        out.p_light_pi = p3i_exact(ctx.p() + wi * (2.0f * sv.scene_radius));
        out.p_light_n = v3s(0.0f);
        return true;
    }
    ShapeSampleContext sctx;
    sctx.pi = ctx.pi; sctx.n = ctx.n; sctx.ns = ctx.ns;
    ShapeSample ss;
    const PrimRec& pr = light_prim_rec(sv, light);
    bool ok;
    if (!TRI_ONLY && (pr.kind_index & PRIM_SPHERE_BIT)) ok = sphere_sample_with_context(sv.spheres[pr.kind_index & PRIM_INDEX_MASK], sctx, u, ss);
    else if (!TRI_ONLY && (pr.kind_index & PRIM_PATCH_BIT)) ok = blp_sample_with_context(load_patch_rec(sv, pr), sctx, u, ss, sv.quirks_off != 0);
    else ok = triangle_sample_with_context(load_triangle_rec(sv, pr), sctx, u, ss, sv.quirks_off != 0);
    if (!ok) return false;
    if (ss.pdf == 0.0f || length_squared(ss.pi.mid() - ctx.p()) == 0.0f) return false;
    V3 wi = normalize(ss.pi.mid() - ctx.p());
    Spec le = area_light_l(sv, light, ss.n, -wi, lambda);
    if (is_zero(le)) return false;
    out.l = le; out.wi = wi; out.pdf = ss.pdf;
    out.p_light_pi = ss.pi;
    out.p_light_n = ss.n;
    return true;
}
template <bool TRI_ONLY = false, bool HAS_TEX = false>
SHM_HD Float light_pdf_li(const SceneView& sv, const ShmLight& light, const LightSampleContext& ctx, V3 wi) {
    if (HAS_TEX && light.kind == SHM_LIGHT_IMAGE_INFINITE) {
        const ImageLightRec& il = sv.image_lights[light.primitive];
        V3 w_light = xf_vector(il.light_from_render, wi);
        V2 uv = equal_area_sphere_to_square(w_light);
        return pc2d_pdf(sv.dist_data, il.compensated, (int)il.n, uv) / (4.0f * PI_F);
    }
    if (light.kind != SHM_LIGHT_DIFFUSE_AREA) return 0.0f;
    ShapeSampleContext sctx;
    sctx.pi = ctx.pi; sctx.n = ctx.n; sctx.ns = ctx.ns;
    const PrimRec& pr = light_prim_rec(sv, light);
    if (!TRI_ONLY && (pr.kind_index & PRIM_SPHERE_BIT)) return sphere_pdf_with_context(sv.spheres[pr.kind_index & PRIM_INDEX_MASK], sctx, wi, sv.quirks_off != 0);
    if (!TRI_ONLY && (pr.kind_index & PRIM_PATCH_BIT)) return blp_pdf_with_context(load_patch_rec(sv, pr), sctx, wi, sv.quirks_off != 0);
    return triangle_pdf_with_context(load_triangle_rec(sv, pr), sctx, wi);
}
template <bool HAS_TEX = false>
SHM_HD Spec infinite_light_le(const SceneView& sv, const ShmLight& light, V3 ray_d, const Wavelengths& lambda) {
    if (HAS_TEX && light.kind == SHM_LIGHT_IMAGE_INFINITE) return light.scale * image_light_le(sv, sv.image_lights[light.primitive], ray_d, lambda);
    return light.scale * spectrum_sample(light.spectrum, sv.spectrum_data, lambda);
}
SHM_HD int light_sampler_sample(const SceneView& sv, Float u, Float& p) {
    if (sv.n_lights == 0) return -1;
    uint32_t idx = (uint32_t)(u * (Float)sv.n_lights);
    if (idx > sv.n_lights - 1) idx = sv.n_lights - 1;
    p = 1.0f / (Float)sv.n_lights;
    return (int)idx;
}
SHM_HD Float light_sampler_pmf(const SceneView& sv) { return sv.n_lights == 0 ? 0.0f : 1.0f / (Float)sv.n_lights; }

template <bool HAS_TEX = false>
SHM_HD BSDF get_bsdf(const SceneView& sv, SurfaceInteraction& si, const ShmMaterial& m_in, Wavelengths& lambda, const Differentials* df = nullptr) {
    TextureEvalContext tctx;
    if (HAS_TEX) tctx = tex_ctx_from(si, *df);
    auto fval = [&](const ShmMaterial& mm, int slot, Float constant) {
        if (HAS_TEX && mm.float_tex[slot] != 0u) return float_texture_evaluate(sv, mm.float_tex[slot] - 1u, tctx);
        return constant;
    };
    const ShmMaterial* mp = &m_in;
    for (int level = 0; mp->kind == SHM_MATERIAL_MIX && level < 16; ++level) {
        Float amt = fval(*mp, SHM_FLOATSLOT_MIX_AMOUNT, mp->mix_amount);
        uint32_t pick;
        if (amt <= 0.0f) pick = 0;
        else if (amt >= 1.0f) pick = 1;
        else {
            uint64_t h = hash_v3(hash_v3(0x4d495800ULL + (uint64_t)level, si.wo), si.p());
            Float u = (Float)(uint32_t)(h >> 40) * 5.9604644775390625e-8f;
            pick = (amt < u) ? 0u : 1u;
        }
        mp = &sv.materials[mp->mix_material[pick]];
    }
    const ShmMaterial& m = *mp;
    if (m.has_displacement) {
        V3 dpdu, dpdv;
        if (HAS_TEX && m.float_tex[SHM_FLOATSLOT_DISPLACEMENT] != 0u) {
            bump_map_texture(sv, m.float_tex[SHM_FLOATSLOT_DISPLACEMENT] - 1u, si, *df, dpdu, dpdv);
        } else {
            Float displace = m.displacement;
            Float du = 0.0005f, dv = 0.0005f;
            dpdu = si.shading.dpdu + (displace - displace) / du * si.shading.n + displace * si.shading.dndu;
            dpdv = si.shading.dpdv + (displace - displace) / dv * si.shading.n + displace * si.shading.dndv;
        }
        V3 ns = normalize(cross(dpdu, dpdv));
        set_shading_geometry(si, ns, dpdu, dpdv, si.shading.dndu, si.shading.dndv, false);
    } else if (HAS_TEX && m.normal_map != 0u) {
        V3 dpdu, dpdv;
        normal_map_texture(sv, m.normal_map - 1u, si, dpdu, dpdv);
        V3 ns = normalize(cross(dpdu, dpdv));
        set_shading_geometry(si, ns, dpdu, dpdv, si.shading.dndu, si.shading.dndv, false);
    }
    auto tex = [&](const ShmSpectrum& s) { return spectrum_texture_evaluate<HAS_TEX>(sv, s, &tctx, lambda); };
    BxDF b;
    b.kind = m.kind;
    b.r = spec_const(0.0f);
    b.k = spec_const(0.0f);
    b.eta = 1.0f;
    b.mf.alpha_x = 0.0f;
    b.mf.alpha_y = 0.0f;
    b.mf2.alpha_x = 0.0f;
    b.mf2.alpha_y = 0.0f;
    b.thickness = 0.0f;
    b.g = 0.0f;
    b.albedo = spec_const(0.0f);
    b.max_depth = 0;
    b.n_samples = 1;
    b.strict = (int)sv.quirks_off;
    if (m.kind == SHM_MATERIAL_DIFFUSE) {
        b.r = clamp(tex(m.a), 0.0f, 1.0f);
    } else if (m.kind == SHM_MATERIAL_CONDUCTOR) {
        Float ur = fval(m, SHM_FLOATSLOT_U_ROUGHNESS, m.u_roughness), vr = fval(m, SHM_FLOATSLOT_V_ROUGHNESS, m.v_roughness);
        if (m.remap_roughness) { ur = roughness_to_alpha(ur); vr = roughness_to_alpha(vr); }
        b.r = tex(m.a);
        b.k = tex(m.b);
        b.mf = trowbridge_reitz_new(ur, vr);
    } else if (m.kind == SHM_MATERIAL_DIELECTRIC) {
        Float sampled_eta = spectrum_get(m.a, sv.spectrum_data, lambda.lambda[0]);
        if (m.a.kind != SHM_SPECTRUM_CONSTANT) terminate_secondary(lambda);
        if (sampled_eta == 0.0f) sampled_eta = 1.0f;
        Float ur = fval(m, SHM_FLOATSLOT_U_ROUGHNESS, m.u_roughness), vr = fval(m, SHM_FLOATSLOT_V_ROUGHNESS, m.v_roughness);
        if (m.remap_roughness) { ur = roughness_to_alpha(ur); vr = roughness_to_alpha(vr); }
        b.eta = sampled_eta;
        b.mf = trowbridge_reitz_new(ur, vr);
    } else if (m.kind == SHM_MATERIAL_THIN_DIELECTRIC) {
        Float sampled_eta = spectrum_get(m.a, sv.spectrum_data, lambda.lambda[0]);
        if (m.a.kind != SHM_SPECTRUM_CONSTANT) terminate_secondary(lambda);
        if (sampled_eta == 0.0f) sampled_eta = 1.0f;
        b.eta = sampled_eta;
    } else if (m.kind == SHM_MATERIAL_COATED_DIFFUSE) {
        b.r = clamp(tex(m.a), 0.0f, 1.0f);
        Float ur = fval(m, SHM_FLOATSLOT_U_ROUGHNESS, m.u_roughness), vr = fval(m, SHM_FLOATSLOT_V_ROUGHNESS, m.v_roughness);
        if (m.remap_roughness) { ur = roughness_to_alpha(ur); vr = roughness_to_alpha(vr); }
        b.mf = trowbridge_reitz_new(ur, vr);
// ... 186 lines not shown
```

### shimmer_amd/csrc/shm/sampling.h

```cpp
#pragma once
#include "vec.h"

namespace shm {

#ifdef SHM_ORACLE_REFERENCE_STREAM
struct RefStream {
    uint64_t s[4];
};
inline uint64_t ref_splitmix64_next(uint64_t& state) {
    state += 0x9e3779b97f4a7c15ULL;
    uint64_t z = state;
    z = (z ^ (z >> 30)) * 0xbf58476d1ce4e5b9ULL;
    z = (z ^ (z >> 27)) * 0x94d049bb133111ebULL;
    return z ^ (z >> 31);
}
inline RefStream ref_stream_seed_from_u64(uint64_t seed) {
    RefStream r;
    for (int i = 0; i < 4; ++i) r.s[i] = ref_splitmix64_next(seed);
    return r;
}
inline uint64_t ref_rotl(uint64_t x, int k) { return (x << k) | (x >> (64 - k)); }
inline uint64_t ref_stream_next_u64(RefStream& r) {
    const uint64_t result = ref_rotl(r.s[0] + r.s[3], 23) + r.s[0];
    const uint64_t t = r.s[1] << 17;
// ... 261 lines not shown
    if (u_remapped) *u_remapped = min((up - sum) / weights[offset], 1.0f - 1.1920929e-7f);
    return offset;
}
SHM_HD Float power_heuristic(int nf, Float f_pdf, int ng, Float g_pdf) {
    Float f = (Float)nf * f_pdf;
    Float g = (Float)ng * g_pdf;
    if (is_inf(sqr(f))) return 1.0f;
    return (f * f) / (f * f + g * g);
}
SHM_HD Float linear_pdf(Float x, Float a, Float b) {
    if (x < 0.0f || x > 1.0f) return 0.0f;
    return 2.0f * lerp(x, a, b) / (a + b);
}
SHM_HD Float sample_linear(Float u, Float a, Float b) {
    if (u == 0.0f && a == 0.0f) return 0.0f;
    Float x = u * (a + b) / (a + sqrt(lerp(u, a * a, b * b)));
    return min(x, 1.0f - FLOAT_EPSILON);
}
SHM_HD V3 sample_uniform_sphere(V2 u) {
    Float z = 1.0f - 2.0f * u.x;
    Float r = safe_sqrt(1.0f - z * z);
    Float phi = 2.0f * PI_F * u.y;
    return v3(r * cos(phi), r * sin(phi), z);
}
SHM_HD V3 sample_uniform_hemisphere(V2 u) {
    Float z = u.x;
    Float r = safe_sqrt(1.0f - z * z);
    Float phi = 2.0f * PI_F * u.y;
    return v3(r * cos(phi), r * sin(phi), z);
}
SHM_HD Float uniform_sphere_pdf() { return INV_4PI; }
SHM_HD Float uniform_hemisphere_pdf(bool strict = false) { return strict ? INV_2PI : INV_4PI; }
SHM_HD V2 sample_uniform_disk_concentric(V2 u) {
    V2 uo = 2.0f * u - v2(1.0f, 1.0f);
    if (uo.x == 0.0f && uo.y == 0.0f) return v2(0.0f, 0.0f);
    Float r, theta;
    if (abs(uo.x) > abs(uo.y)) {
        r = uo.x;
        theta = PI_OVER_4 * (uo.y / uo.x);
    } else {
        r = uo.y;
        theta = PI_OVER_2 - PI_OVER_4 * (uo.x / uo.y);
    }
    return r * v2(cos(theta), sin(theta));
}
SHM_HD V3 sample_cosine_hemisphere(V2 u) {
    V2 d = sample_uniform_disk_concentric(u);
    Float z = safe_sqrt(1.0f - sqr(d.x) - sqr(d.y));
    return v3(d.x, d.y, z);
}
SHM_HD Float cosine_hemisphere_pdf(Float cos_theta) { return cos_theta * INV_PI; }
SHM_HD V2 sample_uniform_disk_polar(V2 u) {
    Float r = sqrt(u.x);
    Float theta = 2.0f * PI_F * u.y;
    return v2(r * cos(theta), r * sin(theta));
}
SHM_HD void sample_uniform_triangle(V2 u, Float& b0, Float& b1, Float& b2) {
    if (u.x < u.y) {
        b0 = u.x / 2.0f;
        b1 = u.y - b0;
    } else {
        b1 = u.y / 2.0f;
        b0 = u.x - b1;
    }
    b2 = 1.0f - b1 - b0;
}
SHM_HD V2 sample_bilinear(V2 u, const Float w[4]) {
    Float y = sample_linear(u.y, w[0] + w[1], w[2] + w[3]);
    Float x = sample_linear(u.x, lerp(y, w[0], w[2]), lerp(y, w[1], w[3]));
    return v2(x, y);
}
SHM_HD Float bilinear_pdf(V2 p, const Float w[4]) {
    if (p.x < 0.0f || p.x > 1.0f || p.y < 0.0f || p.y > 1.0f) return 0.0f;
    if (w[0] + w[1] + w[2] + w[3] == 0.0f) return 1.0f;
    return 4.0f
           * ((1.0f - p.x) * (1.0f - p.y) * w[0] + p.x * (1.0f - p.y) * w[1] + (1.0f - p.x) * p.y * w[2]
              + p.x * p.y * w[3])
           / (w[0] + w[1] + w[2] + w[3]);
}
SHM_HD Float spherical_triangle_area(V3 a, V3 b, V3 c) {
    return abs(2.0f * atan2(dot(a, cross(b, c)), 1.0f + dot(a, b) + dot(a, c) + dot(b, c)));
}

SHM_HD Float sample_spherical_triangle(const V3 v[3], V3 p, V2 u, Float b[3], bool strict = false) {
    V3 a = v[0] - p, bb = v[1] - p, c = v[2] - p;
    a = normalize(a);
    bb = normalize(bb);
    c = normalize(c);
    V3 n_ab = cross(a, bb), n_bc = cross(bb, c), n_ca = cross(c, a);
    if (length_squared(n_ab) == 0.0f || length_squared(n_bc) == 0.0f || length_squared(n_ca) == 0.0f) {
        b[0] = b[1] = b[2] = 0.0f;
        return 0.0f;
    }
    n_ab = normalize(n_ab);
    n_bc = normalize(n_bc);
    n_ca = normalize(n_ca);

    Float alpha = angle_between(n_ab, -n_ca);
    Float beta = angle_between(n_bc, -n_ab);
    Float gamma_ = angle_between(n_ca, -n_bc);

    Float a_pi = alpha + beta + gamma_;
    Float ap_pi = lerp(u.x, PI_F, a_pi);
    Float area = a_pi - PI_F;
    Float pdf = (area <= 0.0f) ? 0.0f : 1.0f / area;

    Float cos_alpha = cos(alpha);
    Float sin_alpha = sin(alpha);
    Float sin_phi = sin(ap_pi) * cos_alpha - cos(ap_pi) * sin_alpha;
    Float cos_phi = cos(ap_pi) * cos_alpha + sin(ap_pi) * sin_alpha;
    Float k1 = cos_phi + cos_alpha;
    Float k2 = sin_phi - sin_alpha * dot(a, bb);
    Float cos_bp = (k2 + (difference_of_products(k2, cos_phi, k1, sin_phi)) * cos_alpha)
                   / (sum_of_products(k2, sin_phi, k1, cos_phi) * sin_alpha);
    cos_bp = clamp(cos_bp, -1.0f, 1.0f);

    Float sin_bp = safe_sqrt(1.0f - cos_bp * cos_bp);
    V3 cp = cos_bp * a + sin_bp * normalize(gram_schmidt(c, a));

    Float cos_theta = 1.0f - u.y * (1.0f - dot(cp, bb));
    Float sin_theta = safe_sqrt(1.0f - cos_theta * cos_theta);
    V3 w = cos_theta * bb + sin_theta * normalize(gram_schmidt(cp, bb));

    V3 e1 = v[1] - v[0];
    V3 e2 = v[2] - v[0];
    V3 s1 = cross(w, e2);
    Float divisor = strict ? dot(s1, e1) : dot(e1, e1);
    if (divisor == 0.0f) {
        b[0] = b[1] = b[2] = 1.0f / 3.0f;
        return pdf;
    }
    Float inv_divisor = 1.0f / divisor;
    V3 s = p - v[0];
    Float b1 = dot(s, s1) * inv_divisor;
    Float b2 = dot(w, cross(s, e1)) * inv_divisor;
    b1 = clamp(b1, 0.0f, 1.0f);
    b2 = clamp(b2, 0.0f, 1.0f);
    if (b1 + b2 > 1.0f) {
        if (strict) {
            b1 = b1 / (b1 + b2);
            b2 = b2 / (b1 + b2);
        } else {
            Float nb1 = b1 / b1 + b2;
            Float nb2 = b2 / b1 + b2;
            b1 = nb1;
            b2 = nb2;
        }
    }
    b[0] = 1.0f - b1 - b2;
    b[1] = b1;
    b[2] = b2;
    return pdf;
}

SHM_HD V2 invert_spherical_triangle_sample(const V3 v[3], V3 p, V3 w) {
    V3 a = normalize(v[0] - p), b = normalize(v[1] - p), c = normalize(v[2] - p);
    V3 n_ab = cross(a, b), n_bc = cross(b, c), n_ca = cross(c, a);
    if (length_squared(n_ab) == 0.0f || length_squared(n_bc) == 0.0f || length_squared(n_ca) == 0.0f)
        return v2(0.0f, 0.0f);
    n_ab = normalize(n_ab);
    n_bc = normalize(n_bc);
    n_ca = normalize(n_ca);
    Float alpha = angle_between(n_ab, -n_ca);
    Float beta = angle_between(n_bc, -n_ab);
    Float gamma_ = angle_between(n_ca, -n_bc);

    V3 cp = normalize(cross(cross(b, w), cross(c, a)));
    if (dot(cp, a + c) < 0.0f) cp = -cp;

    Float u0;
    if (dot(a, cp) > 0.99999847691f) {
        u0 = 0.0f;
    } else {
        V3 n_cpb = cross(cp, b);
        V3 n_acp = cross(a, cp);
        if (length_squared(n_cpb) == 0.0f || length_squared(n_acp) == 0.0f) return v2(0.5f, 0.5f);
        n_cpb = normalize(n_cpb);
        n_acp = normalize(n_acp);
        Float ap = alpha + angle_between(n_ab, n_cpb) + angle_between(n_acp, -n_cpb) - PI_F;
        Float area = alpha + beta + gamma_ - PI_F;
        u0 = ap / area;
    }
    Float u1 = (1.0f - dot(w, b)) / (1.0f - dot(cp, b));
    return v2(clamp(u0, 0.0f, 1.0f), clamp(u1, 0.0f, 1.0f));
}

}
```

### shimmer_amd/csrc/shm/scene.h

```cpp
#pragma once
#include <assert.h>
#include "shapes.h"
#include "patch.h"
#include "spectrum.h"

namespace shm {

struct PrimRec {
    Float p0[3], p1[3], p2[3];
    uint32_t kind_index;
    uint32_t mesh;
    uint32_t tri;
    uint32_t material;
    int32_t area_light;
    uint32_t pad[2];
};
static_assert(sizeof(PrimRec) == 64, "PrimRec is one aligned 64-byte record");
struct PatchExtra {
    Float p11[3];
    Float area;
    uint32_t flags;
    uint32_t pad[3];
};
static_assert(sizeof(PatchExtra) == 32, "PatchExtra must be 32 bytes");
constexpr uint32_t PRIM_PATCH_BIT = 0x40000000u;
constexpr uint32_t PRIM_INSTANCE_BIT = 0x20000000u;
constexpr uint32_t PRIM_DEGENERATE_BIT = 0x10000000u;
constexpr uint32_t PRIM_INDEX_MASK = 0x0fffffffu;
constexpr uint32_t PRIM_SPHERE_BIT = 0x80000000u;

enum : uint32_t { MESH_HAS_N = 1, MESH_HAS_S = 2, MESH_HAS_UV = 4, MESH_FLIP = 8 };

struct SceneView {
    const ShmBvhNode* nodes;
    uint32_t n_nodes;
    const PrimRec* prim_recs;
    const ShmPrimitive* primitives;
    uint32_t n_primitives;
    const uint32_t* mesh_flags;
    const uint32_t* vi;
    const Float* vn;
    const Float* vs;
    const Float* vuv;
    const ShmSphere* spheres;
    const PatchExtra* patches;
    const uint32_t* patch_vi;
    const Float* patch_vn;
    const Float* patch_vuv;
    const ShmMaterial* materials;
    const ShmLight* lights;
    uint32_t n_lights;
    const struct PrimRec* light_prim_recs;
    const uint32_t* infinite_lights;
    uint32_t n_infinite_lights;
    const Float* spectrum_data;
    Float scene_radius;
    ShmCamera camera;
    int32_t pixel_bounds[4];
    Float filter_radius[2];
    Float imaging_ratio;
    Float max_component_value;
    uint32_t filter_kind;
    const Float* sensor_r_bar;
    const Float* sensor_g_bar;
    const Float* sensor_b_bar;
    const ShmImageTexture* image_textures;
    const ShmImageLevel* image_levels;
    const Float* texel_data;
    uint32_t rgb2spec_res;
    const Float* rgb2spec_scale;
    const Float* rgb2spec_data;
    const Float* cs_illuminant;
    const Float* ewa_lut;
    const ShmInstance* instances;
    const ShmFloatTexture* float_textures;
    const struct FloatTexRange* ftex_ranges;
    const struct FloatTexOp* ftex_ops;
    const ShmSpectrumTexture* spectrum_textures;
    const struct FloatTexRange* stex_ranges;
    const struct FloatTexOp* stex_ops;
    const struct ImageLightRec* image_lights;
    const Float* dist_data;
    uint32_t quirks_off;
    uint32_t zsobol;
    const SceneView* call_copy;
    const ShmBvhNode* inst_roots;
    const struct TriShadeRec* tri_shade;
};

constexpr int FTEX_MAX_OPS = 32;
constexpr int STEX_MAX_OPS = 8;
struct FloatTexOp {
    uint32_t node;
    uint8_t a, b, c, pad;
};
struct FloatTexRange {
    uint32_t first, count;
};

struct Dist2DRec {
    uint32_t func, cdf, marginal_func, marginal_cdf;
    Float marginal_int;
    uint32_t pad[3];
};
struct ImageLightRec {
    Float render_from_light[16];
    Float light_from_render[16];
    uint32_t image_level;
    uint32_t n;
    uint32_t pad[2];
    Dist2DRec distribution, compensated;
};

SHM_HD V3 ld3(const Float* p) { return v3(p[0], p[1], p[2]); }

SHM_HD TriangleData load_triangle_rec(const SceneView& sv, const PrimRec& pr) {
    TriangleData t;
    t.p0 = ld3(pr.p0);
    t.p1 = ld3(pr.p1);
    t.p2 = ld3(pr.p2);
    uint32_t f = sv.mesh_flags[pr.mesh];
    t.has_n = (f & MESH_HAS_N) != 0;
    t.has_s = (f & MESH_HAS_S) != 0;
    t.has_uv = (f & MESH_HAS_UV) != 0;
    t.flip = (f & MESH_FLIP) != 0;
    t.uv0 = t.uv1 = t.uv2 = v2(0.0f, 0.0f);
    t.n0 = t.n1 = t.n2 = v3s(0.0f);
    t.s0 = t.s1 = t.s2 = v3s(0.0f);
    if (f & (MESH_HAS_N | MESH_HAS_S | MESH_HAS_UV)) {
        uint32_t i0 = sv.vi[3 * pr.tri], i1 = sv.vi[3 * pr.tri + 1], i2 = sv.vi[3 * pr.tri + 2];
        if (t.has_n) { t.n0 = ld3(sv.vn + 3 * i0); t.n1 = ld3(sv.vn + 3 * i1); t.n2 = ld3(sv.vn + 3 * i2); }
        if (t.has_s) { t.s0 = ld3(sv.vs + 3 * i0); t.s1 = ld3(sv.vs + 3 * i1); t.s2 = ld3(sv.vs + 3 * i2); }
        if (t.has_uv) {
            t.uv0 = v2(sv.vuv[2 * i0], sv.vuv[2 * i0 + 1]);
            t.uv1 = v2(sv.vuv[2 * i1], sv.vuv[2 * i1 + 1]);
            t.uv2 = v2(sv.vuv[2 * i2], sv.vuv[2 * i2 + 1]);
        }
    }
    return t;
}
SHM_HD TriangleData load_triangle(const SceneView& sv, uint32_t slot) { return load_triangle_rec(sv, sv.prim_recs[slot]); }
SHM_HD const PrimRec& light_prim_rec(const SceneView& sv, const ShmLight& light) {
#if !defined(__HIP_DEVICE_COMPILE__)
    assert(&light >= sv.lights && &light < sv.lights + sv.n_lights);
#endif
    return sv.light_prim_recs ? sv.light_prim_recs[&light - sv.lights] : sv.prim_recs[light.primitive];
}
SHM_HD const PrimRec& light_side_rec(const SceneView& sv, const ShmLight& light) {
#if !defined(__HIP_DEVICE_COMPILE__)
    assert(&light >= sv.lights && &light < sv.lights + sv.n_lights && sv.light_prim_recs);
#endif
    return sv.light_prim_recs[&light - sv.lights];
}

SHM_HD PatchData load_patch_rec(const SceneView& sv, const PrimRec& pr) {
    const PatchExtra& px = sv.patches[pr.kind_index & PRIM_INDEX_MASK];
    PatchData pd;
    pd.p00 = ld3(pr.p0); pd.p10 = ld3(pr.p1); pd.p01 = ld3(pr.p2); pd.p11 = ld3(px.p11);
    pd.is_rect = (px.flags & 1u) != 0;
    pd.flip = (px.flags & 2u) != 0;
    pd.area = px.area;
    pd.has_n = (px.flags & 4u) != 0;
    pd.has_uv = (px.flags & 8u) != 0;
    pd.n00 = pd.n10 = pd.n01 = pd.n11 = v3s(0.0f);
    pd.uv00 = pd.uv10 = pd.uv01 = pd.uv11 = v2(0.0f, 0.0f);
    if (px.flags & 12u) {
        const uint32_t* vi = sv.patch_vi + 4u * (pr.kind_index & PRIM_INDEX_MASK);
        if (pd.has_n) { pd.n00 = ld3(sv.patch_vn + 3 * vi[0]); pd.n10 = ld3(sv.patch_vn + 3 * vi[1]); pd.n01 = ld3(sv.patch_vn + 3 * vi[2]); pd.n11 = ld3(sv.patch_vn + 3 * vi[3]); }
        if (pd.has_uv) {
            pd.uv00 = v2(sv.patch_vuv[2 * vi[0]], sv.patch_vuv[2 * vi[0] + 1]);
            pd.uv10 = v2(sv.patch_vuv[2 * vi[1]], sv.patch_vuv[2 * vi[1] + 1]);
            pd.uv01 = v2(sv.patch_vuv[2 * vi[2]], sv.patch_vuv[2 * vi[2] + 1]);
            pd.uv11 = v2(sv.patch_vuv[2 * vi[3]], sv.patch_vuv[2 * vi[3] + 1]);
        }
    }
    return pd;
}

SHM_HD PatchData load_patch(const SceneView& sv, uint32_t slot) { return load_patch_rec(sv, sv.prim_recs[slot]); }

struct Hit {
    int32_t prim;
    Float t;
    Float b0, b1, b2;
    Float phi;
    int32_t inst = -1;
};

SHM_HD Ray xf_ray_inverse(const Float* minv, V3 ro, V3 rd, Float& t_max) {
    P3i o = xf_point_i(minv, p3i_exact(ro));
    V3 d = xf_vector(minv, rd);
    Float ls = length_squared(d);
    if (ls > 0.0f) {
        V3 o_error = v3(o.x.width() / 2.0f, o.y.width() / 2.0f, o.z.width() / 2.0f);
        Float dt = dot(abs3(d), o_error) / ls;
        t_max = t_max - dt;
        o = o + p3i_exact(d * dt);
    }
    Ray r;
    r.o = o.mid();
    r.d = d;
    return r;
}

template <bool TRI_ONLY = false>
SHM_HD SurfaceInteraction hit_interaction_local(const SceneView& sv, const Hit& h, V3 wo);
template <bool TRI_ONLY = false>
SHM_HD SurfaceInteraction hit_interaction(const SceneView& sv, const Hit& h, V3 wo) {
    if (!TRI_ONLY && h.inst >= 0) {
        const ShmInstance& in = sv.instances[sv.prim_recs[h.inst].kind_index & PRIM_INDEX_MASK];
        V3 wo_local = xf_vector(in.primitive_from_render, wo);
        return xf_surface_interaction(in.render_from_primitive, in.primitive_from_render, hit_interaction_local<false>(sv, h, wo_local), sv.quirks_off != 0);
    }
    return hit_interaction_local<TRI_ONLY>(sv, h, wo);
}
template <bool TRI_ONLY>
SHM_HD SurfaceInteraction hit_interaction_local(const SceneView& sv, const Hit& h, V3 wo) {
    const PrimRec& pr = sv.prim_recs[h.prim];
    if (!TRI_ONLY && (pr.kind_index & PRIM_SPHERE_BIT)) {
        QuadricIntersection qi;
        qi.t_hit = h.t;
        qi.p_obj = v3(h.b0, h.b1, h.b2);
        qi.phi = h.phi;
        return sphere_interaction(sv.spheres[pr.kind_index & PRIM_INDEX_MASK], qi, wo, sv.quirks_off != 0);
    }
    if (!TRI_ONLY && (pr.kind_index & PRIM_PATCH_BIT)) return blp_interaction(load_patch(sv, (uint32_t)h.prim), h.b0, h.b1, wo);
    TriangleData tr = load_triangle(sv, (uint32_t)h.prim);
    TriangleIntersection ti;
    ti.b0 = h.b0; ti.b1 = h.b1; ti.b2 = h.b2; ti.t = h.t;
    return triangle_interaction(tr, ti, wo);
}

SHM_HD bool prim_intersect(const SceneView& sv, uint32_t slot, V3 ro, V3 rd, Float t_max, Hit& h) {
    const PrimRec& pr = sv.prim_recs[slot];
    if (pr.kind_index & PRIM_SPHERE_BIT) {
        QuadricIntersection qi;
        if (!sphere_basic_intersect(sv.spheres[pr.kind_index & PRIM_INDEX_MASK], ro, rd, t_max, qi)) return false;
        h.prim = (int32_t)slot; h.t = qi.t_hit; h.b0 = qi.p_obj.x; h.b1 = qi.p_obj.y; h.b2 = qi.p_obj.z; h.phi = qi.phi;
        return true;
    }
    if (pr.kind_index & PRIM_PATCH_BIT) {
        BilinearIntersection bi;
        if (!blp_intersect(ro, rd, t_max, ld3(pr.p0), ld3(pr.p1), ld3(pr.p2), ld3(sv.patches[pr.kind_index & PRIM_INDEX_MASK].p11), bi)) return false;
        h.prim = (int32_t)slot; h.t = bi.t; h.b0 = bi.u; h.b1 = bi.v; h.b2 = 0.0f; h.phi = 0.0f;
        return true;
    }
    TriangleIntersection ti;
    if (!intersect_triangle(ro, rd, t_max, ld3(pr.p0), ld3(pr.p1), ld3(pr.p2), ti)) return false;
    h.prim = (int32_t)slot; h.t = ti.t; h.b0 = ti.b0; h.b1 = ti.b1; h.b2 = ti.b2; h.phi = 0.0f;
    return true;
}

}
```

### shimmer_amd/csrc/shm/shapes.h

```cpp
#pragma once
#include "sampling.h"
#include "../../../include/shimmer_hip.h"

namespace shm {

struct Ray {
    V3 o, d;
};

SHM_HD bool intersect_p_cached(const Float bmin[3], const Float bmax[3], V3 o, Float ray_t_max, V3 inv_dir,
                               const int dir_is_neg[3]) {
    const Float g = 1.0f + 2.0f * gamma(3);
    Float t_min = ((dir_is_neg[0] ? bmax[0] : bmin[0]) - o.x) * inv_dir.x;
    Float t_max = ((dir_is_neg[0] ? bmin[0] : bmax[0]) - o.x) * inv_dir.x;
    Float ty_min = ((dir_is_neg[1] ? bmax[1] : bmin[1]) - o.y) * inv_dir.y;
    Float ty_max = ((dir_is_neg[1] ? bmin[1] : bmax[1]) - o.y) * inv_dir.y;
    t_max *= g;
    ty_max *= g;
    if (t_min > ty_max || ty_min > t_max) return false;
    if (ty_min > t_min) t_min = ty_min;
    if (ty_max < t_max) t_max = ty_max;
    Float tz_min = ((dir_is_neg[2] ? bmax[2] : bmin[2]) - o.z) * inv_dir.z;
    Float tz_max = ((dir_is_neg[2] ? bmin[2] : bmax[2]) - o.z) * inv_dir.z;
    tz_max *= g;
// ... 396 lines not shown
    Interval q;
    if (b.midpoint() < 0.0f) q = -0.5f * (b - root_discrim);
    else q = -0.5f * (b + root_discrim);
    Interval t0 = q / a;
    Interval t1 = c / q;
    if (t0.low > t1.low) { Interval tmp = t0; t0 = t1; t1 = tmp; }
    if (t0.high > t_max || t1.low <= 0.0f) return false;
    Interval t_shape_hit = t0;
    if (t_shape_hit.low <= 0.0f) {
        t_shape_hit = t1;
        if (t_shape_hit.high > t_max) return false;
    }
    V3 p_hit = oi.mid() + t_shape_hit.midpoint() * di.mid();
    p_hit = p_hit * (s.radius / distance(p_hit, v3s(0.0f)));
    if (p_hit.x == 0.0f && p_hit.y == 0.0f) p_hit.x = 1e-5f * s.radius;
    Float phi = atan2(p_hit.y, p_hit.x);
    if (phi < 0.0f) phi += 2.0f * PI_F;
    if ((s.z_min > -s.radius && p_hit.z < s.z_min) || (s.z_max < s.radius && p_hit.z > s.z_max)
        || phi > s.phi_max) {
        if (t_shape_hit == t1) return false;
        if (t1.high > t_max) return false;
        t_shape_hit = t1;
        p_hit = oi.mid() + t_shape_hit.midpoint() * di.mid();
        p_hit = p_hit * (s.radius / distance(p_hit, v3s(0.0f)));
        if (p_hit.x == 0.0f && p_hit.y == 0.0f) p_hit.x = 1e-5f * s.radius;
        phi = atan2(p_hit.y, p_hit.x);
        if (phi < 0.0f) phi += 2.0f * PI_F;
        if ((s.z_min > -s.radius && p_hit.z < s.z_min) || (s.z_max < s.radius && p_hit.z > s.z_max)
            || phi > s.phi_max)
            return false;
    }
    out.t_hit = t_shape_hit.midpoint();
    out.p_obj = p_hit;
    out.phi = phi;
    return true;
}

SHM_HD SurfaceInteraction sphere_interaction(const ShmSphere& s, const QuadricIntersection& isect, V3 wo, bool strict = false) {
    V3 p_hit = isect.p_obj;
    Float phi = isect.phi;
    Float u = phi / s.phi_max;
    Float cos_theta_ = p_hit.z / s.radius;
    Float theta = strict ? acos(clamp(cos_theta_, -1.0f, 1.0f)) : safe_acos(cos_theta_);
    Float v = (theta - s.theta_z_min) / (s.theta_z_max - s.theta_z_min);
    Float z_radius = sqrt(p_hit.x * p_hit.x + p_hit.y * p_hit.y);
    Float cos_phi_ = p_hit.x / z_radius;
    Float sin_phi_ = p_hit.y / z_radius;
    V3 dpdu = v3(-s.phi_max * p_hit.y, s.phi_max * p_hit.x, 0.0f);
    Float sin_theta_ = safe_sqrt(1.0f - cos_theta_ * cos_theta_);
    V3 dpdv = (s.theta_z_max - s.theta_z_min) * v3(p_hit.z * cos_phi_, p_hit.z * sin_phi_, -s.radius * sin_theta_);
    V3 d2pduu = -s.phi_max * s.phi_max * v3(p_hit.x, p_hit.y, 0.0f);
    V3 d2pduv = (s.theta_z_max - s.theta_z_min) * p_hit.z * s.phi_max * v3(-sin_phi_, cos_phi_, 0.0f);
    V3 d2pdvv = -((s.theta_z_max - s.theta_z_min) * (s.theta_z_max - s.theta_z_min)) * v3(p_hit.x, p_hit.y, p_hit.z);
    Float e1 = dot(dpdu, dpdu);
    Float f1 = dot(dpdu, dpdv);
    Float g1 = dot(dpdv, dpdv);
    V3 n = normalize(cross(dpdu, dpdv));
    Float e = dot(n, d2pduu);
    Float f = dot(n, d2pduv);
    Float g = dot(n, d2pdvv);
    Float egf2 = difference_of_products(e1, g1, f1, f1);
    Float env_egf2 = (egf2 == 0.0f) ? 0.0f : 1.0f / egf2;
    V3 dndu = (f * f1 - e * g1) * env_egf2 * dpdu + (e * f1 - f * e1) * env_egf2 * dpdv;
    V3 dndv = (g * f1 - f * g1) * env_egf2 * dpdu + (f * f1 - g * e1) * env_egf2 * dpdv;
    V3 p_error = gamma(5) * abs3(p_hit);
    bool flip_normal = (s.reverse_orientation != 0) ^ (s.transform_swaps_handedness != 0);
    V3 wo_object = xf_vector(s.object_from_render, wo);
    SurfaceInteraction si = surface_interaction_new(p3i_from_value_and_error(p_hit, p_error), v2(u, v), wo_object,
                                                    dpdu, dpdv, dndu, dndv, flip_normal);
    return xf_surface_interaction(s.render_from_object, s.object_from_render, si, strict);
}

struct ShapeSampleContext {
    P3i pi;
    V3 n, ns;
    SHM_HD V3 p() const { return pi.mid(); }
};
struct ShapeSample {
    P3i pi;
    V3 n;
    Float pdf;
};

SHM_HD Float triangle_area(const TriangleData& tr) { return 0.5f * length(cross(tr.p1 - tr.p0, tr.p2 - tr.p0)); }
SHM_HD Float triangle_solid_angle(const TriangleData& tr, V3 p) {
    return spherical_triangle_area(normalize(tr.p0 - p), normalize(tr.p1 - p), normalize(tr.p2 - p));
}
SHM_HD ShapeSample triangle_sample(const TriangleData& tr, V2 u, bool strict = false) {
    Float b0, b1, b2;
    sample_uniform_triangle(u, b0, b1, b2);
    V3 p = b0 * tr.p0 + b1 * tr.p1 + b2 * tr.p2;
    V3 n = normalize(cross(tr.p1 - tr.p0, tr.p2 - tr.p0));
    if (!tr.has_n) {
        if (!strict || tr.flip) n = n * -1.0f;
    } else {
        V3 ns = b0 * tr.n0 + b1 * tr.n1 + b2 * tr.n2;
        n = face_forward(n, ns);
    }
    V3 p_abs_sum = abs3(b0 * tr.p0) + abs3(b1 * tr.p1) + abs3(b2 * tr.p2);
    V3 p_error = gamma(6) * p_abs_sum;
    ShapeSample ss;
    ss.pi = p3i_from_value_and_error(p, p_error);
    ss.n = n;
    ss.pdf = 1.0f / triangle_area(tr);
    return ss;
}
constexpr Float MIN_SPHERICAL_SAMPLE_AREA = 3e-4f;
constexpr Float MAX_SPHERICAL_SAMPLE_AREA = 6.22f;
SHM_HD bool triangle_sample_with_context(const TriangleData& tr, const ShapeSampleContext& ctx, V2 u, ShapeSample& out, bool strict = false) {
    Float solid_angle = triangle_solid_angle(tr, ctx.p());
    if (solid_angle < MIN_SPHERICAL_SAMPLE_AREA || solid_angle > MAX_SPHERICAL_SAMPLE_AREA) {
        ShapeSample ss = triangle_sample(tr, u, strict);
        V3 wi = ss.pi.mid() - ctx.p();
        if (length_squared(wi) == 0.0f) return false;
        wi = normalize(wi);
        ss.pdf /= abs_dot(ss.n, -wi) / distance_squared(ctx.p(), ss.pi.mid());
        if (is_inf(ss.pdf)) return false;
        out = ss;
        return true;
    }
    Float pdf = 1.0f;
    if (ctx.ns != v3s(0.0f)) {
        V3 rp = ctx.p();
        V3 wi0 = normalize(tr.p0 - rp), wi1 = normalize(tr.p1 - rp), wi2 = normalize(tr.p2 - rp);
        Float w[4] = {max(0.01f, abs_dot(ctx.ns, wi1)), max(0.01f, abs_dot(ctx.ns, wi1)),
                      max(0.01f, abs_dot(ctx.ns, wi0)), max(0.01f, abs_dot(ctx.ns, wi2))};
        V2 uw = sample_bilinear(u, w);
        pdf = bilinear_pdf(uw, w);
        if (strict) u = uw;
    }
    V3 verts[3] = {tr.p0, tr.p1, tr.p2};
    Float b[3];
    Float tri_pdf = sample_spherical_triangle(verts, ctx.p(), u, b, strict);
    if (tri_pdf == 0.0f) return false;
    pdf = pdf * tri_pdf;
    V3 p_abs_sum = abs3(b[0] * tr.p0) + abs3(b[1] * tr.p1) + abs3((1.0f - b[0] - b[1]) * tr.p2);
    V3 p_error = gamma(6) * p_abs_sum;
    V3 p = b[0] * tr.p0 + b[1] * tr.p1 + b[2] * tr.p2;
    V3 n = normalize(cross(tr.p1 - tr.p0, tr.p2 - tr.p0));
    if (tr.has_n) {
        V3 ns = b[0] * tr.n0 + b[1] * tr.n1 + b[2] * tr.n2;
        n = face_forward(n, ns);
    } else if (tr.flip) {
        n = n * -1.0f;
    }
    out.pi = p3i_from_value_and_error(p, p_error);
    out.n = n;
    out.pdf = pdf;
    return true;
}
SHM_HD Float triangle_pdf_with_context(const TriangleData& tr, const ShapeSampleContext& ctx, V3 wi) {
    Float solid_angle = triangle_solid_angle(tr, ctx.p());
    if (solid_angle < MIN_SPHERICAL_SAMPLE_AREA || solid_angle > MAX_SPHERICAL_SAMPLE_AREA) {
        V3 o = offset_ray_origin(ctx.pi, ctx.n, wi);
        TriangleIntersection ti;
        if (!intersect_triangle(o, wi, infinity(), tr.p0, tr.p1, tr.p2, ti)) return 0.0f;
        SurfaceInteraction isect = triangle_interaction(tr, ti, -wi);
        Float pdf = (1.0f / triangle_area(tr)) / (abs_dot(isect.n, -wi) / distance_squared(ctx.p(), isect.p()));
        if (is_inf(pdf)) return 0.0f;
        return pdf;
    }
    Float pdf = 1.0f / solid_angle;
    if (ctx.ns != v3s(0.0f)) {
        V3 verts[3] = {tr.p0, tr.p1, tr.p2};
        V2 u = invert_spherical_triangle_sample(verts, ctx.p(), wi);
        V3 rp = ctx.p();
        V3 wi0 = normalize(tr.p0 - rp), wi1 = normalize(tr.p1 - rp), wi2 = normalize(tr.p2 - rp);
        Float w[4] = {max(0.01f, abs_dot(ctx.ns, wi1)), max(0.01f, abs_dot(ctx.ns, wi1)),
                      max(0.01f, abs_dot(ctx.ns, wi0)), max(0.01f, abs_dot(ctx.ns, wi2))};
        pdf *= bilinear_pdf(u, w);
    }
    return pdf;
}

SHM_HD Float sphere_area(const ShmSphere& s) { return s.phi_max * s.radius * (s.z_max - s.z_min); }
SHM_HD ShapeSample sphere_sample(const ShmSphere& s, V2 u) {
    V3 p_obj = v3s(0.0f) + sample_uniform_sphere(u) * s.radius;
    p_obj = p_obj * (s.radius / distance(p_obj, v3s(0.0f)));
    V3 p_obj_error = gamma(5) * abs3(p_obj);
    V3 n_obj = p_obj;
    Float normal_sign = s.reverse_orientation ? -1.0f : 1.0f;
    V3 n = normal_sign * normalize(xf_normal(s.object_from_render, n_obj));
    ShapeSample ss;
    ss.pi = xf_point_i(s.render_from_object, p3i_from_value_and_error(p_obj, p_obj_error));
    ss.n = n;
    ss.pdf = 1.0f / sphere_area(s);
    return ss;
}
SHM_HD bool sphere_sample_with_context(const ShmSphere& s, const ShapeSampleContext& ctx, V2 u, ShapeSample& out) {
    V3 p_center = xf_point(s.render_from_object, v3s(0.0f));
    V3 p_origin = offset_ray_origin(ctx.pi, ctx.n, p_center - ctx.p());
    if (distance_squared(p_origin, p_center) <= sqr(s.radius)) {
        ShapeSample ss = sphere_sample(s, u);
        V3 wi = ss.pi.mid() - ctx.p();
        if (length_squared(wi) == 0.0f) return false;
        wi = normalize(wi);
        ss.pdf /= abs_dot(ss.n, -wi) / distance_squared(ctx.p(), ss.pi.mid());
        if (is_inf(ss.pdf)) return false;
        out = ss;
        return true;
    }
    Float sin_theta_max = s.radius / distance(ctx.p(), p_center);
    Float sin2_theta_max = sqr(sin_theta_max);
    Float cos_theta_max = safe_sqrt(1.0f - sin2_theta_max);
    Float one_minus_cos_theta_max = 1.0f - cos_theta_max;
    Float cos_theta_ = (cos_theta_max - 1.0f) * u.x + 1.0f;
    Float sin2_theta_ = 1.0f - sqr(cos_theta_);
    if (sin2_theta_max < 0.00068523f) {
        sin2_theta_ = sin2_theta_max * u.x;
        cos_theta_ = sqrt(1.0f - sin2_theta_);
        one_minus_cos_theta_max = sin2_theta_max / 2.0f;
    }
    Float cos_alpha = sin2_theta_ / sin_theta_max + cos_theta_ * safe_sqrt(1.0f - sin2_theta_ / sqr(sin_theta_max));
    Float sin_alpha = safe_sqrt(1.0f - sqr(cos_alpha));
    Float phi = u.y * 2.0f * PI_F;
    V3 w = spherical_direction(sin_alpha, cos_alpha, phi);
    Frame sampling_frame = frame_from_z(normalize(p_center - ctx.p()));
    Float normal_sign = s.reverse_orientation ? -1.0f : 1.0f;
    V3 n = normal_sign * sampling_frame.from_local(-w);
    V3 p = p_center + v3(n.x, n.y, n.z) * s.radius;
    V3 p_error = gamma(5) * abs3(p);
    out.pi = p3i_from_value_and_error(p, p_error);
    out.n = n;
    out.pdf = 1.0f / (2.0f * PI_F * one_minus_cos_theta_max);
    return true;
}
SHM_HD Float sphere_pdf_with_context(const ShmSphere& s, const ShapeSampleContext& ctx, V3 wi, bool strict = false) {
    V3 p_center = xf_point(s.render_from_object, v3s(0.0f));
    V3 p_origin = offset_ray_origin(ctx.pi, ctx.n, p_center - ctx.p());
    if (distance_squared(p_origin, p_center) <= s.radius * s.radius) {
        V3 o = offset_ray_origin(ctx.pi, ctx.n, wi);
        QuadricIntersection qi;
        if (!sphere_basic_intersect(s, o, wi, infinity(), qi)) return 0.0f;
        SurfaceInteraction isect = sphere_interaction(s, qi, -wi);
        Float pdf = strict ? (1.0f / sphere_area(s)) / (abs_dot(isect.n, -wi) / distance_squared(ctx.p(), isect.p()))
                           : (1.0f / sphere_area(s)) / abs_dot(isect.n, -wi) / distance_squared(ctx.p(), isect.p());
        if (is_inf(pdf)) return 0.0f;
        return pdf;
    }
    Float sin2_theta_max = s.radius * s.radius / distance_squared(ctx.p(), p_center);
    Float cos_theta_max = safe_sqrt(1.0f - sin2_theta_max);
    Float one_minus_cos_theta_max = 1.0f - cos_theta_max;
    if (sin2_theta_max < 0.00068523f) one_minus_cos_theta_max = sin2_theta_max / 2.0f;
    return 1.0f / ((strict ? 2.0f : 2.90f) * PI_F * one_minus_cos_theta_max);
}

}
```

### shimmer_amd/csrc/wavefront.h

```cpp
#pragma once
#include <hip/hip_runtime.h>
#include <stdio.h>
#include <stdlib.h>
#include <string.h>

#include <algorithm>
#include <string>
#include <vector>

#include "host/flatten.h"
#include "shm/bvh_link.h"
#include "host/bvh_pairs.hpp"
#include "host/render_plan.hpp"
#ifndef K_DELTA_LIGHTS
#define K_DELTA_LIGHTS false
#endif
#define SHM_DELTA_LIGHTS K_DELTA_LIGHTS
#define SHM_DIFFUSE_TRANSMISSION K_DELTA_LIGHTS
#ifndef K_SPHERICAL_CAMERA
#define K_SPHERICAL_CAMERA false
#endif
#define SHM_SPHERICAL_CAMERA K_SPHERICAL_CAMERA
#include "shm/path.h"
#include "shm/tri_shade.h"
#define WF_CAT_(a, b) a##b
#define WF_CAT(a, b) WF_CAT_(a, b)
#if K_DELTA_LIGHTS
#define WF_DL_NAME(name) WF_CAT(name, _dl)
#else
#define WF_DL_NAME(name) name
#endif

using namespace shm;

__attribute__((visibility("hidden"))) std::string& shm_err();

namespace wf {

#define HIP_TRY(expr)                                                                            \
    do {                                                                                         \
        hipError_t _e = (expr);                                                                  \
        if (_e != hipSuccess) {                                                                  \
            shm_err() = std::string(#expr) + ": " + hipGetErrorString(_e);                           \
            (void)hipGetLastError();  \
            return SHM_ERR_DEVICE;                                                               \
        }                                                                                        \
    } while (0)

#define LAUNCH_TRY(what)                                                                         \
    do {                                                                                         \
        hipError_t _e = hipGetLastError();                                                       \
        if (_e != hipSuccess) {                                                                  \
            shm_err() = std::string("launch of ") + (what) + ": " + hipGetErrorString(_e);           \
            return SHM_ERR_DEVICE;                                                               \
        }                                                                                        \
    } while (0)

static inline bool dbg_on() { static int v = -1; if (v < 0) v = getenv("SHM_DEBUG") ? 1 : 0; return v == 1; }
#define DBG(...) do { if (dbg_on()) { fprintf(stderr, "[shm] " __VA_ARGS__); fprintf(stderr, "\n"); fflush(stderr); } } while (0)

constexpr int WAVE = 64;
constexpr int TRACE_BLOCK = 256;
constexpr int SHADE_BLOCK = 128;
constexpr uint32_t TRACE_QUEUE_PARTS = 8, TRACE_HEAD_STRIDE = 32;

constexpr uint32_t HIT_HAS_SECOND = 0x40000000u;

struct DeviceCounters {
    unsigned long long rays_closest, rays_any, nodes_closest, tris_closest, nodes_any, tris_any, paths;
};

struct QueueState {
    uint32_t n_active[2];
    uint32_t n_shadow[2];
    uint32_t n_scatter[4];
    uint32_t n_lean;
    uint32_t n_emit;
    uint32_t n_split;
};

struct alignas(64) PathRec {
    float4 lambda;
    uint2 rng;
    uint32_t pixel;
    uint32_t flags;
    float4 beta;
    float2 pb_eta;
    uint32_t pad[2];
};
static_assert(sizeof(PathRec) == 64, "PathRec is one half cache line");
#ifndef K_ZSOBOL
#define K_ZSOBOL false
#endif
template <bool ZS = K_ZSOBOL>
__device__ __forceinline__ uint32_t sampler_word(const SceneView& sv) {
    return ZS ? sv.zsobol : 0u;
}
__device__ __forceinline__ Rng sampler_load(uint2 rs, uint32_t pix, const SceneView& sv, const ShmRenderParams& params) {
    return sampler_resume((uint64_t)rs.x | ((uint64_t)rs.y << 32), pix & 0xffffu, pix >> 16, params.seed, sampler_word(sv));
}
__device__ __forceinline__ uint2 sampler_store(const Rng& r) {
    const uint64_t w = sampler_save(r);
    return make_uint2((uint32_t)w, (uint32_t)(w >> 32));
}
struct alignas(128) BxRec {
    float4 bx0;
    float4 bx2;
    float4 fr;
    float4 bx1;
    float4 bx3;
    float4 bx4;
    float4 siwo;
    float4 pad;
};
static_assert(sizeof(BxRec) == 128, "BxRec is one cache line");
struct alignas(64) CtxRec { float4 c0, c1, c2, pad; };
struct PathArrays {
    ShmRay* ray;
    ShmHit* hit;
    const float4* hit_prev;
    uint32_t hit16;
    ShmRay* shadow_ray;
    float4* shadow_contrib;
    float4* L;
    PathRec* rec;
    float4* lambda;
    uint2* rng0;
    uint32_t* pixel0;
    float4* lambda_pdf;
    CtxRec* ctx;
    float4* aux0;
    float4* aux1;
    float4* aux2;
    BxRec* bx;
    uint32_t has_layered;
    const float4* hit2;
    float4* dd0;
    float4* dd1;
    float4* dd2;
    float4* e_ray;
    float4* e_beta;
    float4* e_ctx0;
    float4* e_ctx1;
    float4* e_ctx2;
    uint32_t* e_flags;
};
enum : int { CLASS_DIFFUSE = 0, CLASS_CONDUCTOR = 1, CLASS_DIELECTRIC = 2, CLASS_LAYERED = 3, N_BXDF_CLASSES = 4 };
__device__ inline int bxdf_class_of(uint32_t kind) {
    if (SHM_DIFFUSE_TRANSMISSION && kind == SHM_MATERIAL_DIFFUSE_TRANSMISSION) return CLASS_DIFFUSE;
    return kind == SHM_MATERIAL_DIFFUSE ? CLASS_DIFFUSE : (kind == SHM_MATERIAL_CONDUCTOR ? CLASS_CONDUCTOR : (kind <= SHM_MATERIAL_THIN_DIELECTRIC ? CLASS_DIELECTRIC : CLASS_LAYERED));
}

__device__ __forceinline__ AuxRays ld_aux(const PathArrays& pa, uint32_t path) {
    float4 a = pa.aux0[path], b = pa.aux1[path], c = pa.aux2[path];
    AuxRays x;
    x.has = true;
    x.rx_o = v3(a.x, a.y, a.z); x.rx_d = v3(a.w, b.x, b.y);
    x.ry_o = v3(b.z, b.w, c.x); x.ry_d = v3(c.y, c.z, c.w);
    return x;
}
__device__ __forceinline__ void st_aux(const PathArrays& pa, uint32_t path, const AuxRays& x) {
    pa.aux0[path] = make_float4(x.rx_o.x, x.rx_o.y, x.rx_o.z, x.rx_d.x);
    pa.aux1[path] = make_float4(x.rx_d.y, x.rx_d.z, x.ry_o.x, x.ry_o.y);
    pa.aux2[path] = make_float4(x.ry_o.z, x.ry_d.x, x.ry_d.y, x.ry_d.z);
}

constexpr uint32_t LDS_TABLE_BUDGET = 12 * 1024, LDS_TABLE_BUDGET_SMALL = 1536;
enum : int { LT_MESH_FLAGS, LT_LIGHTS, LT_LIGHT_PRIMS, LT_MATERIALS, LT_SPECTRUM, LT_RGB2SPEC_SCALE, LT_IMAGE_TEXTURES, LT_IMAGE_LEVELS, LT_FLOAT_TEXTURES, LT_FTEX_RANGES, LT_FTEX_OPS, LT_SPECTRUM_TEXTURES,
              LT_STEX_RANGES, LT_STEX_OPS, LT_EWA_LUT, N_LDS_TABLES };
struct LdsTables {
    uint32_t bytes[N_LDS_TABLES];
};
__device__ __forceinline__ SceneView stage_scene_tables(const SceneView& sv, const LdsTables& t, uint4* lds) {
    SceneView out = sv;
    uint32_t total = 0;
#pragma unroll
    for (int k = 0; k < N_LDS_TABLES; ++k) total += t.bytes[k];
    if (total == 0u) return out;
    uint32_t at = 0;
#define SHM_STAGE_TABLE(K, FIELD, TYPE)                                                                \
    if (t.bytes[K]) {                                                                                  \
        const uint32_t n = t.bytes[K] / 16u;                                                           \
        const uint4* g = reinterpret_cast<const uint4*>(sv.FIELD);                                     \
        for (uint32_t i = threadIdx.x; i < n; i += blockDim.x) lds[at + i] = g[i];                     \
        out.FIELD = reinterpret_cast<const TYPE*>(lds + at);                                           \
        at += n;                                                                                       \
    }
    SHM_STAGE_TABLE(LT_MESH_FLAGS, mesh_flags, uint32_t)
    SHM_STAGE_TABLE(LT_LIGHTS, lights, ShmLight)
    SHM_STAGE_TABLE(LT_LIGHT_PRIMS, light_prim_recs, PrimRec)
    SHM_STAGE_TABLE(LT_MATERIALS, materials, ShmMaterial)
    SHM_STAGE_TABLE(LT_SPECTRUM, spectrum_data, Float)
    SHM_STAGE_TABLE(LT_RGB2SPEC_SCALE, rgb2spec_scale, Float)
    SHM_STAGE_TABLE(LT_IMAGE_TEXTURES, image_textures, ShmImageTexture)
    SHM_STAGE_TABLE(LT_IMAGE_LEVELS, image_levels, ShmImageLevel)
    SHM_STAGE_TABLE(LT_FLOAT_TEXTURES, float_textures, ShmFloatTexture)
    SHM_STAGE_TABLE(LT_FTEX_RANGES, ftex_ranges, FloatTexRange)
    SHM_STAGE_TABLE(LT_FTEX_OPS, ftex_ops, FloatTexOp)
    SHM_STAGE_TABLE(LT_SPECTRUM_TEXTURES, spectrum_textures, ShmSpectrumTexture)
    SHM_STAGE_TABLE(LT_STEX_RANGES, stex_ranges, FloatTexRange)
    SHM_STAGE_TABLE(LT_STEX_OPS, stex_ops, FloatTexOp)
    SHM_STAGE_TABLE(LT_EWA_LUT, ewa_lut, Float)
#undef SHM_STAGE_TABLE
    __syncthreads();
    return out;
}

constexpr uint32_t SCENE_VIEW_UINT4S = (sizeof(SceneView) + 15) / 16;
__device__ __forceinline__ void attach_call_copy(SceneView& sv, uint4* slot) {
    SceneView* call_copy = reinterpret_cast<SceneView*>(slot);
    sv.call_copy = call_copy;
    if (threadIdx.x == 0) *call_copy = sv;
    __syncthreads();
}
template <bool HAS_TEX>
__device__ __forceinline__ SceneView stage_scene_tables_tex(const SceneView& sv, const LdsTables& t, uint4* lds, uint4* slot) {
    SceneView out = stage_scene_tables(sv, t, lds);
    if (HAS_TEX) attach_call_copy(out, slot);
    return out;
}

__device__ __forceinline__ int hit_prim_of(int w) { return w < 0 ? w : (int)((uint32_t)w & ~HIT_HAS_SECOND); }
__device__ __forceinline__ Hit load_hit_tri(const PathArrays& pa, uint32_t path) {
    Hit hit;
    if (pa.hit16) {
        const float4 h = reinterpret_cast<const float4*>(pa.hit)[path];
        const int w = __float_as_int(h.x);
        hit.prim = hit_prim_of(w); hit.t = 0.0f; hit.b0 = h.y; hit.b1 = h.z; hit.b2 = h.w; hit.phi = 0.0f; hit.inst = -1;
        if (w >= 0 && ((uint32_t)w & HIT_HAS_SECOND)) {
            const float4 h2 = pa.hit2[path];
            hit.t = h2.x; hit.phi = h2.y;
        }
    } else {
        const float4* hp = reinterpret_cast<const float4*>(pa.hit + path);
        const float4 h0 = hp[0], h1 = hp[1];
        hit.prim = __float_as_int(h0.x); hit.t = h0.y; hit.b0 = h0.z; hit.b1 = h0.w; hit.b2 = h1.x; hit.phi = h1.y; hit.inst = __float_as_int(h1.z) - 1;
    }
    return hit;
}

__device__ __forceinline__ uint32_t wave_lane() { return __lane_id(); }

__device__ __forceinline__ uint32_t queue_push_slot(uint32_t* counter, bool pred) {
    unsigned long long mask = __ballot(pred);
    if (mask == 0ull) return 0u;
    uint32_t lane = wave_lane();
    int leader = __ffsll((long long)mask) - 1;
    uint32_t base = 0;
    if ((int)lane == leader) base = atomicAdd(counter, (uint32_t)__popcll(mask));
    base = __shfl(base, leader);
    uint32_t rank = (uint32_t)__popcll(mask & ((1ull << lane) - 1ull));
    return base + rank;
}
__device__ __forceinline__ Spec ld_spec(const float4& f) { Spec s; s.v[0] = f.x; s.v[1] = f.y; s.v[2] = f.z; s.v[3] = f.w; return s; }
__device__ __forceinline__ float4 st_spec(const Spec& s) { return make_float4(s.v[0], s.v[1], s.v[2], s.v[3]); }
constexpr int SHADE2_BLOCK = 256;
constexpr int SHADE_CHUNK = 2048;
#ifndef K_SHADE_WAVES
#define K_SHADE_WAVES 2
#endif
#define K_SHADE_ATTR __attribute__((amdgpu_waves_per_eu(K_SHADE_WAVES, K_SHADE_WAVES)))
}
using namespace wf;

struct TraceSide {
    int blocks = 0;
    int spill_levels = 1;
    uint32_t* d_spill = nullptr;
    float4* d_gen_save = nullptr;
    uint32_t* d_heads = nullptr;
};
struct ShmScene {
    int device = 0;
    hipStream_t stream = nullptr;
    shm_host::FlatScene flat;
    SceneView dsv;
    shm_plan::ScenePlan plan;
    std::vector<void*> allocs;
    std::vector<void*> ws_allocs;
    ShmFilmPixel* d_film = nullptr;
    size_t n_film_pixels = 0;
    uint32_t capacity = 0;
    PathArrays pa;
    uint32_t* d_q_active[2] = {nullptr, nullptr};
    uint32_t* d_q_shadow = nullptr;
// ... 126 lines not shown
```

Measured before the change: 5137.

## Precompute per-light triangle and patch sampling records on host and stage in LDS

Builds a 128-byte per-light sample record (normals, inverse area, edge lengths, rectangle frame, bilinear weights) on the host, uploads it, and optionally stages it into LDS. Light sampling and pdf code in the wavefront kernels then reads these records instead of recomputing cross products, normalizations and areas on every shadow sample. A host probe is added to compare the record and non-record paths. This adds memory traffic and LDS budget pressure from a 128-byte-per-light table, which may push other tables out of LDS in scenes with many emissive primitives.

```diff
diff --git a/include/shimmer_hip.h b/include/shimmer_hip.h
--- a/include/shimmer_hip.h
+++ b/include/shimmer_hip.h
@@ -464,6 +464,8 @@
 SHM_API int shm_bvh_build(const float* prim_bounds, uint32_t n, int split_method, ShmBvhNode* nodes_out,
                   uint32_t* n_nodes_out, uint32_t* prim_order_out);
 SHM_API int shm_bounds3_probe(const float a[6], const float b[6], const float p[3], float out[16]);
+SHM_API int shm_light_sample_records_probe(const ShmSceneDesc* desc, uint32_t light, int disable_reference_quirks, uint32_t n, const float* ctx, const float* u,
+                                           const float* wi, float* out);
 SHM_API int shm_tile_bounds(const int32_t pixel_bounds[4], int32_t tile_w, int32_t tile_h, ShmTile* tiles_out,
                     uint32_t* n_out);
 SHM_API int shm_camera_perspective(const float world_from_camera[16], float fov_deg, const int32_t full_resolution[2],
diff --git a/shimmer_amd/abi.py b/shimmer_amd/abi.py
--- a/shimmer_amd/abi.py
+++ b/shimmer_amd/abi.py
@@ -250,6 +250,7 @@
     "shm_device_count": (C.c_int, []),
     "shm_bvh_build": (C.c_int, [c_float_p, C.c_uint32, C.c_int, C.POINTER(ShmBvhNode), c_u32_p, c_u32_p]),
     "shm_bounds3_probe": (C.c_int, [c_float_p, c_float_p, c_float_p, c_float_p]),
+    "shm_light_sample_records_probe": (C.c_int, [C.POINTER(ShmSceneDesc), C.c_uint32, C.c_int, C.c_uint32, c_float_p, c_float_p, c_float_p, c_float_p]),
     "shm_tile_bounds": (C.c_int, [C.POINTER(C.c_int32), C.c_int32, C.c_int32, C.POINTER(ShmTile), c_u32_p]),
     "shm_camera_perspective": (C.c_int, [c_float_p, C.c_float, C.POINTER(C.c_int32), C.c_float, C.c_float, C.POINTER(ShmCamera), c_float_p]),
     "shm_integrator_render": (C.c_int, [C.c_char_p, C.POINTER(ShmSceneDesc), C.c_int, C.c_int32, C.c_int, C.c_int, C.c_int, C.c_int32, C.c_int32, C.c_int, C.c_int,
diff --git a/shimmer_amd/csrc/host/flatten.h b/shimmer_amd/csrc/host/flatten.h
--- a/shimmer_amd/csrc/host/flatten.h
+++ b/shimmer_amd/csrc/host/flatten.h
@@ -71,6 +71,8 @@
         v.call_copy = nullptr;
         v.inst_roots = nullptr;
         v.tri_shade = nullptr;
+        v.light_sample_recs = nullptr;
+        v.inv_n_lights = 0.0f;
         v.nodes = nodes.data();
         v.n_nodes = (uint32_t)nodes.size();
         v.prim_recs = prim_recs.data();
@@ -722,4 +724,11 @@
     return SHM_OK;
 }
 
+inline std::vector<shm::LightSampleRec> build_light_sample_recs(const FlatScene& f) {
+    const shm::SceneView v = f.view();
+    std::vector<shm::LightSampleRec> recs(f.lights.size());
+    for (size_t i = 0; i < recs.size(); ++i) recs[i] = shm::light_sample_rec_of(v, f.lights[i]);
+    return recs;
 }
+
+}
diff --git a/shimmer_amd/csrc/host/host_mirror.cpp b/shimmer_amd/csrc/host/host_mirror.cpp
--- a/shimmer_amd/csrc/host/host_mirror.cpp
+++ b/shimmer_amd/csrc/host/host_mirror.cpp
@@ -12,6 +12,7 @@
 
 #include "../../../include/shimmer_hip.h"
 #include "../shm/path.h"
+#include "flatten.h"
 
 extern "C" __attribute__((visibility("hidden"))) void shm_set_last_error(const char* msg);
 
@@ -243,6 +244,45 @@
     out[13] = (ba.mx[0] - ba.mn[0]) * (ba.mx[1] - ba.mn[1]) * (ba.mx[2] - ba.mn[2]);
     out[14] = (float)b3_max_dimension(ba);
     out[15] = 0.0f;
+    return SHM_OK;
+}
+
+int shm_light_sample_records_probe(const ShmSceneDesc* desc, uint32_t light, int disable_reference_quirks, uint32_t n, const float* ctx, const float* u, const float* wi,
+                                   float* out) {
+    if (!desc || !ctx || !u || !wi || !out) return SHM_ERR_INVALID_ARGUMENT;
+    shm_host::FlatScene flat;
+    std::string err;
+    const int rc = shm_host::flatten_scene(desc, flat, err);
+    if (rc != SHM_OK) { shm_set_last_error(err.c_str()); return rc; }
+    if (light >= flat.lights.size()) { shm_set_last_error("light index out of range"); return SHM_ERR_INVALID_ARGUMENT; }
+    const std::vector<shm::LightSampleRec> recs = shm_host::build_light_sample_recs(flat);
+    shm::SceneView views[2] = {flat.view(), flat.view()};
+    views[1].light_sample_recs = recs.data();
+    views[1].inv_n_lights = shm::light_sampler_inv_n(views[0]);
+    const shm::Wavelengths lambda = shm::sample_visible(0.5f);
+    for (uint32_t i = 0; i < n; ++i) {
+        shm::LightSampleContext c;
+        c.pi = shm::p3i_exact(shm::v3(ctx[9 * i], ctx[9 * i + 1], ctx[9 * i + 2]));
+        c.n = shm::v3(ctx[9 * i + 3], ctx[9 * i + 4], ctx[9 * i + 5]);
+        c.ns = shm::v3(ctx[9 * i + 6], ctx[9 * i + 7], ctx[9 * i + 8]);
+        for (int k = 0; k < 2; ++k) {
+            shm::SceneView& sv = views[k];
+            sv.quirks_off = disable_reference_quirks ? 1u : 0u;
+            float* o = out + ((size_t)i * 2 + k) * 20;
+            for (int j = 0; j < 20; ++j) o[j] = 0.0f;
+            shm::LightLiSample ls;
+            if (shm::light_sample_li<false, true>(sv, sv.lights[light], c, shm::v2(u[2 * i], u[2 * i + 1]), lambda, ls)) {
+                o[0] = 1.0f;
+                for (int j = 0; j < 4; ++j) o[1 + j] = ls.l.v[j];
+                o[5] = ls.wi.x; o[6] = ls.wi.y; o[7] = ls.wi.z; o[8] = ls.pdf;
+                o[9] = ls.p_light_pi.x.low; o[10] = ls.p_light_pi.y.low; o[11] = ls.p_light_pi.z.low;
+                o[12] = ls.p_light_pi.x.high; o[13] = ls.p_light_pi.y.high; o[14] = ls.p_light_pi.z.high;
+                o[15] = ls.p_light_n.x; o[16] = ls.p_light_n.y; o[17] = ls.p_light_n.z;
+            }
+            o[18] = shm::light_pdf_li<false, true>(sv, sv.lights[light], c, shm::v3(wi[3 * i], wi[3 * i + 1], wi[3 * i + 2]));
+            o[19] = shm::light_sampler_pmf(sv);
+        }
+    }
     return SHM_OK;
 }
 
diff --git a/shimmer_amd/csrc/render.hip b/shimmer_amd/csrc/render.hip
--- a/shimmer_amd/csrc/render.hip
+++ b/shimmer_amd/csrc/render.hip
@@ -254,7 +254,8 @@
         pad16(f.rgb2spec_scale.size() * sizeof(float)),
         pad16(f.image_textures.size() * sizeof(ShmImageTexture)), pad16(f.image_levels.size() * sizeof(ShmImageLevel)), pad16(f.float_textures.size() * sizeof(ShmFloatTexture)),
         pad16(f.ftex_ranges.size() * sizeof(shm::FloatTexRange)), pad16(f.ftex_ops.size() * sizeof(shm::FloatTexOp)), pad16(f.spectrum_textures.size() * sizeof(ShmSpectrumTexture)),
-        pad16(f.stex_ranges.size() * sizeof(shm::FloatTexRange)), pad16(f.stex_ops.size() * sizeof(shm::FloatTexOp)), pad16(f.ewa_lut.size() * sizeof(float))};
+        pad16(f.stex_ranges.size() * sizeof(shm::FloatTexRange)), pad16(f.stex_ops.size() * sizeof(shm::FloatTexOp)), pad16(f.ewa_lut.size() * sizeof(float)),
+        pad16(f.lights.size() * sizeof(shm::LightSampleRec))};
     size_t left = budget;
     for (int k = 0; k < N_LDS_TABLES; ++k)
         if (want[k] && want[k] <= left) { t.bytes[k] = (uint32_t)want[k]; left -= want[k]; }
@@ -330,6 +331,8 @@
     UP(f.materials, materials); UP(f.lights, lights);
     v.light_prim_recs = nullptr;
     if (!f.light_prim_recs.empty()) UP(f.light_prim_recs, light_prim_recs);
+    UP(shm_host::build_light_sample_recs(f), light_sample_recs);
+    v.inv_n_lights = v.n_lights ? light_sampler_inv_n(v) : 0.0f;
     UP(f.infinite_lights, infinite_lights); UP(f.spectrum_data, spectrum_data); UP(f.sensor_r, sensor_r_bar); UP(f.sensor_g, sensor_g_bar); UP(f.sensor_b, sensor_b_bar);
     UP(f.image_textures, image_textures); UP(f.image_levels, image_levels); UP(f.texel_data, texel_data); UP(f.rgb2spec_scale, rgb2spec_scale);
     UP(f.rgb2spec_data, rgb2spec_data); UP(f.cs_illuminant, cs_illuminant); UP(f.ewa_lut, ewa_lut);
diff --git a/shimmer_amd/csrc/shm/patch.h b/shimmer_amd/csrc/shm/patch.h
--- a/shimmer_amd/csrc/shm/patch.h
+++ b/shimmer_amd/csrc/shm/patch.h
@@ -218,12 +218,51 @@
     return abs(alpha + beta + gamma_ + delta - 2.0f * PI_F);
 }
 
-SHM_HD V3 sample_spherical_rectangle(V3 p_ref, V3 s, V3 ex, V3 ey, V2 u, Float& pdf) {
-    Float exl = length(ex), eyl = length(ey);
+struct RectSampleRec {
+    Float exl, eyl;
+    V3 rx, ry, rz;
+};
+SHM_HD RectSampleRec rect_sample_rec(V3 ex, V3 ey) {
+    RectSampleRec r;
+    r.exl = length(ex);
+    r.eyl = length(ey);
+    r.rx = ex / r.exl;
+    r.ry = ey / r.eyl;
+    r.rz = cross(r.rx, r.ry);
+    return r;
+}
+struct alignas(16) PatchSampleRec {
+    V3 eu, ev;
+    RectSampleRec rect;
+    V3 n;
+    Float d2u, d2v;
+    Float w[4];
+    Float pad[6];
+};
+static_assert(sizeof(PatchSampleRec) == 128, "PatchSampleRec is two 64-byte slots");
+SHM_HD PatchSampleRec patch_sample_rec(V3 p00, V3 p10, V3 p01, V3 p11) {
+    PatchSampleRec r;
+    r.eu = p10 - p00;
+    r.ev = p01 - p00;
+    r.rect = rect_sample_rec(r.eu, r.ev);
+    r.n = normalize(cross(r.eu, r.ev));
+    r.d2u = distance_squared(p10, p00);
+    r.d2v = distance_squared(p01, p00);
+    r.w[0] = length(cross(p10 - p00, p01 - p00));
+    r.w[1] = length(cross(p10 - p00, p11 - p10));
+    r.w[2] = length(cross(p01 - p00, p11 - p01));
+    r.w[3] = length(cross(p11 - p10, p11 - p01));
+    for (int i = 0; i < 6; ++i) r.pad[i] = 0.0f;
+    return r;
+}
+SHM_HD PatchSampleRec patch_sample_rec(const PatchData& pd) { return patch_sample_rec(pd.p00, pd.p10, pd.p01, pd.p11); }
+
+SHM_HD V3 sample_spherical_rectangle(V3 p_ref, V3 s, V3 ex, V3 ey, const RectSampleRec& rc, V2 u, Float& pdf) {
+    Float exl = rc.exl, eyl = rc.eyl;
     Frame r;
-    r.x = ex / exl;
-    r.y = ey / eyl;
-    r.z = cross(r.x, r.y);
+    r.x = rc.rx;
+    r.y = rc.ry;
+    r.z = rc.rz;
     V3 d_local = r.to_local(s - p_ref);
     Float z0 = d_local.z;
     if (z0 > 0.0f) {
@@ -257,13 +296,16 @@
     Float yv = (hvsq < 1.0f - 1e-6f) ? (hv * dd) / sqrt(1.0f - hvsq) : y1;
     return p_ref + r.from_local(v3(xu, yv, z0));
 }
-
-SHM_HD V2 invert_spherical_rectangle_sample(V3 p_ref, V3 s, V3 ex, V3 ey, V3 p_rect) {
-    Float exl = length(ex), eyl = length(ey);
+SHM_HD V3 sample_spherical_rectangle(V3 p_ref, V3 s, V3 ex, V3 ey, V2 u, Float& pdf) {
+    return sample_spherical_rectangle(p_ref, s, ex, ey, rect_sample_rec(ex, ey), u, pdf);
+}
+
+SHM_HD V2 invert_spherical_rectangle_sample(V3 p_ref, V3 s, V3 ex, V3 ey, const RectSampleRec& rc, V3 p_rect) {
+    Float exl = rc.exl, eyl = rc.eyl;
     Frame r;
-    r.x = ex / exl;
-    r.y = ey / eyl;
-    r.z = cross(r.x, r.y);
+    r.x = rc.rx;
+    r.y = rc.ry;
+    r.z = rc.rz;
     V3 d_local = r.to_local(s - p_ref);
     Float z0 = d_local.z;
     if (z0 > 0.0f) {
@@ -308,18 +350,19 @@
     if (abs(yza - yv) < abs(yzb - yv)) return v2(clamp(u0, 0.0f, 1.0f), u1a);
     return v2(clamp(u0, 0.0f, 1.0f), u1b);
 }
-
-SHM_HD bool blp_sample(const PatchData& pd, V2 u, ShapeSample& out, bool strict = false) {
+SHM_HD V2 invert_spherical_rectangle_sample(V3 p_ref, V3 s, V3 ex, V3 ey, V3 p_rect) {
+    return invert_spherical_rectangle_sample(p_ref, s, ex, ey, rect_sample_rec(ex, ey), p_rect);
+}
+
+SHM_HD bool blp_sample(const PatchData& pd, const PatchSampleRec& rc, V2 u, ShapeSample& out, bool strict = false) {
     V2 uv;
     Float pdf;
     if (pd.is_rect) {
         uv = u;
         pdf = 1.0f;
     } else {
-        Float w[4] = {length(cross(pd.p10 - pd.p00, pd.p01 - pd.p00)), length(cross(pd.p10 - pd.p00, pd.p11 - pd.p10)),
-                      length(cross(pd.p01 - pd.p00, pd.p11 - pd.p01)), length(cross(pd.p11 - pd.p10, pd.p11 - pd.p01))};
-        uv = sample_bilinear(u, w);
-        pdf = bilinear_pdf(uv, w);
+        uv = sample_bilinear(u, rc.w);
+        pdf = bilinear_pdf(uv, rc.w);
     }
     V3 pu0 = strict ? lerp3(uv.y, pd.p00, pd.p01) : lerp3(uv.x, pd.p00, pd.p10);
     V3 pu1 = lerp3(uv.y, pd.p10, pd.p11);
@@ -337,29 +380,27 @@
     out.pdf = pdf / length(cross(dpdu, dpdv));
     return true;
 }
-SHM_HD Float blp_pdf(const PatchData& pd, V2 uv, bool strict = false) {
+SHM_HD bool blp_sample(const PatchData& pd, V2 u, ShapeSample& out, bool strict = false) { return blp_sample(pd, patch_sample_rec(pd), u, out, strict); }
+SHM_HD Float blp_pdf(const PatchData& pd, const PatchSampleRec& rc, V2 uv, bool strict = false) {
     if (pd.has_uv) uv = invert_bilinear(uv, pd.uv00, pd.uv10, pd.uv01, pd.uv11);
     Float pdf = 1.0f;
-    if (!pd.is_rect) {
-        Float w[4] = {length(cross(pd.p10 - pd.p00, pd.p01 - pd.p00)), length(cross(pd.p10 - pd.p00, pd.p11 - pd.p10)),
-                      length(cross(pd.p01 - pd.p00, pd.p11 - pd.p01)), length(cross(pd.p11 - pd.p10, pd.p11 - pd.p01))};
-        pdf = bilinear_pdf(uv, w);
-    }
+    if (!pd.is_rect) pdf = bilinear_pdf(uv, rc.w);
     V3 pu0 = strict ? lerp3(uv.y, pd.p00, pd.p01) : lerp3(uv.y, pd.p00, pd.p10);
     V3 pu1 = lerp3(uv.y, pd.p10, pd.p11);
     V3 dpdu = pu1 - pu0;
     V3 dpdv = lerp3(uv.x, pd.p01, pd.p11) - lerp3(uv.x, pd.p00, pd.p10);
     return pdf / length(cross(dpdu, dpdv));
 }
+SHM_HD Float blp_pdf(const PatchData& pd, V2 uv, bool strict = false) { return blp_pdf(pd, patch_sample_rec(pd), uv, strict); }
 
 constexpr Float BLP_MIN_SPHERICAL_SAMPLE_AREA = 1e-4f;
 
-SHM_HD bool blp_sample_with_context(const PatchData& pd, const ShapeSampleContext& ctx, V2 u, ShapeSample& out, bool strict = false) {
+SHM_HD bool blp_sample_with_context(const PatchData& pd, const PatchSampleRec& rc, const ShapeSampleContext& ctx, V2 u, ShapeSample& out, bool strict = false) {
     V3 rp = ctx.p();
     V3 v00 = normalize(pd.p00 - rp), v10 = normalize(pd.p10 - rp), v01 = normalize(pd.p01 - rp), v11 = normalize(pd.p11 - rp);
     if (!pd.is_rect || spherical_quad_area(v00, v10, v11, v01) <= BLP_MIN_SPHERICAL_SAMPLE_AREA) {
         ShapeSample ss;
-        if (!blp_sample(pd, u, ss, strict)) return false;
+        if (!blp_sample(pd, rc, u, ss, strict)) return false;
         V3 wi = ss.pi.mid() - rp;
         if (length_squared(wi) == 0.0f) return false;
         wi = normalize(wi);
@@ -374,12 +415,12 @@
         u = sample_bilinear(u, w);
         pdf = bilinear_pdf(u, w);
     }
-    V3 eu = pd.p10 - pd.p00, ev = pd.p01 - pd.p00;
+    V3 eu = rc.eu, ev = rc.ev;
     Float quad_pdf = 0.0f;
-    V3 p = sample_spherical_rectangle(rp, pd.p00, eu, ev, u, quad_pdf);
+    V3 p = sample_spherical_rectangle(rp, pd.p00, eu, ev, rc.rect, u, quad_pdf);
     pdf *= quad_pdf;
-    V2 uv = v2(dot(p - pd.p00, eu) / distance_squared(pd.p10, pd.p00), dot(p - pd.p00, ev) / distance_squared(pd.p01, pd.p00));
-    V3 n = normalize(cross(eu, ev));
+    V2 uv = v2(dot(p - pd.p00, eu) / rc.d2u, dot(p - pd.p00, ev) / rc.d2v);
+    V3 n = rc.n;
     if (pd.has_n) n = face_forward(n, blp_interp_normal(pd, uv.x, uv.y));
     else if (pd.flip) n = -n;
     out.pi = p3i_exact(p);
@@ -387,8 +428,11 @@
     out.pdf = pdf;
     return true;
 }
-
-SHM_HD Float blp_pdf_with_context(const PatchData& pd, const ShapeSampleContext& ctx, V3 wi, bool strict = false) {
+SHM_HD bool blp_sample_with_context(const PatchData& pd, const ShapeSampleContext& ctx, V2 u, ShapeSample& out, bool strict = false) {
+    return blp_sample_with_context(pd, patch_sample_rec(pd), ctx, u, out, strict);
+}
+
+SHM_HD Float blp_pdf_with_context(const PatchData& pd, const PatchSampleRec& rc, const ShapeSampleContext& ctx, V3 wi, bool strict = false) {
     V3 o = offset_ray_origin(ctx.pi, ctx.n, wi);
     BilinearIntersection bi;
     if (!blp_intersect(o, wi, infinity(), pd.p00, pd.p10, pd.p01, pd.p11, bi)) return 0.0f;
@@ -396,16 +440,19 @@
     V3 rp = ctx.p();
     V3 v00 = normalize(pd.p00 - rp), v10 = normalize(pd.p10 - rp), v01 = normalize(pd.p01 - rp), v11 = normalize(pd.p11 - rp);
     if (!pd.is_rect || spherical_quad_area(v00, v10, v11, v01) <= BLP_MIN_SPHERICAL_SAMPLE_AREA) {
-        Float pdf = blp_pdf(pd, isect.uv, strict) * distance_squared(rp, isect.p()) / abs_dot(isect.n, -wi);
+        Float pdf = blp_pdf(pd, rc, isect.uv, strict) * distance_squared(rp, isect.p()) / abs_dot(isect.n, -wi);
         return is_inf(pdf) ? 0.0f : pdf;
     }
     Float pdf = 1.0f / spherical_quad_area(v00, v10, v11, v01);
     if (ctx.ns != v3s(0.0f)) {
         Float w[4] = {max(0.01f, dot(v00, ctx.ns)), max(0.01f, dot(v10, ctx.ns)), max(0.01f, dot(v01, ctx.ns)), max(0.01f, dot(v11, ctx.ns))};
-        V2 u = invert_spherical_rectangle_sample(rp, pd.p00, pd.p10 - pd.p00, pd.p01 - pd.p00, isect.p());
+        V2 u = invert_spherical_rectangle_sample(rp, pd.p00, rc.eu, rc.ev, rc.rect, isect.p());
         return bilinear_pdf(u, w) * pdf;
     }
     return pdf;
 }
-
-}
+SHM_HD Float blp_pdf_with_context(const PatchData& pd, const ShapeSampleContext& ctx, V3 wi, bool strict = false) {
+    return blp_pdf_with_context(pd, patch_sample_rec(pd), ctx, wi, strict);
+}
+
+}
diff --git a/shimmer_amd/csrc/shm/path.h b/shimmer_amd/csrc/shm/path.h
--- a/shimmer_amd/csrc/shm/path.h
+++ b/shimmer_amd/csrc/shm/path.h
@@ -26,6 +26,10 @@
 
 #ifndef SHM_DELTA_LIGHTS
 #define SHM_DELTA_LIGHTS 1
+#endif
+
+#ifndef SHM_LIGHT_SAMPLE_RECS
+#define SHM_LIGHT_SAMPLE_RECS 0
 #endif
 
 SHM_HD bool light_is_delta(const ShmLight& l) {
@@ -115,10 +119,15 @@
     sctx.pi = ctx.pi; sctx.n = ctx.n; sctx.ns = ctx.ns;
     ShapeSample ss;
     const PrimRec& pr = light_prim_rec(sv, light);
+    const LightSampleRec* rc = light_sample_rec(sv, light);
+    const bool recs = SHM_LIGHT_SAMPLE_RECS || rc != nullptr;
     bool ok;
     if (!TRI_ONLY && (pr.kind_index & PRIM_SPHERE_BIT)) ok = sphere_sample_with_context(sv.spheres[pr.kind_index & PRIM_INDEX_MASK], sctx, u, ss);
-    else if (!TRI_ONLY && (pr.kind_index & PRIM_PATCH_BIT)) ok = blp_sample_with_context(load_patch_rec(sv, pr), sctx, u, ss, sv.quirks_off != 0);
-    else ok = triangle_sample_with_context(load_triangle_rec(sv, pr), sctx, u, ss, sv.quirks_off != 0);
+    else if (!TRI_ONLY && (pr.kind_index & PRIM_PATCH_BIT)) {
+        ok = recs ? blp_sample_with_context(load_patch_rec(sv, pr), rc->patch, sctx, u, ss, sv.quirks_off != 0) : blp_sample_with_context(load_patch_rec(sv, pr), sctx, u, ss, sv.quirks_off != 0);
+    } else {
+        ok = recs ? triangle_sample_with_context(load_triangle_rec(sv, pr), rc->tri, sctx, u, ss, sv.quirks_off != 0) : triangle_sample_with_context(load_triangle_rec(sv, pr), sctx, u, ss, sv.quirks_off != 0);
+    }
     if (!ok) return false;
     if (ss.pdf == 0.0f || length_squared(ss.pi.mid() - ctx.p()) == 0.0f) return false;
     V3 wi = normalize(ss.pi.mid() - ctx.p());
@@ -141,23 +150,27 @@
     ShapeSampleContext sctx;
     sctx.pi = ctx.pi; sctx.n = ctx.n; sctx.ns = ctx.ns;
     const PrimRec& pr = light_prim_rec(sv, light);
+    const LightSampleRec* rc = light_sample_rec(sv, light);
+    const bool recs = SHM_LIGHT_SAMPLE_RECS || rc != nullptr;
     if (!TRI_ONLY && (pr.kind_index & PRIM_SPHERE_BIT)) return sphere_pdf_with_context(sv.spheres[pr.kind_index & PRIM_INDEX_MASK], sctx, wi, sv.quirks_off != 0);
-    if (!TRI_ONLY && (pr.kind_index & PRIM_PATCH_BIT)) return blp_pdf_with_context(load_patch_rec(sv, pr), sctx, wi, sv.quirks_off != 0);
-    return triangle_pdf_with_context(load_triangle_rec(sv, pr), sctx, wi);
+    if (!TRI_ONLY && (pr.kind_index & PRIM_PATCH_BIT))
+        return recs ? blp_pdf_with_context(load_patch_rec(sv, pr), rc->patch, sctx, wi, sv.quirks_off != 0) : blp_pdf_with_context(load_patch_rec(sv, pr), sctx, wi, sv.quirks_off != 0);
+    return recs ? triangle_pdf_with_context(load_triangle_rec(sv, pr), rc->tri, sctx, wi) : triangle_pdf_with_context(load_triangle_rec(sv, pr), sctx, wi);
 }
 template <bool HAS_TEX = false>
 SHM_HD Spec infinite_light_le(const SceneView& sv, const ShmLight& light, V3 ray_d, const Wavelengths& lambda) {
     if (HAS_TEX && light.kind == SHM_LIGHT_IMAGE_INFINITE) return light.scale * image_light_le(sv, sv.image_lights[light.primitive], ray_d, lambda);
     return light.scale * spectrum_sample(light.spectrum, sv.spectrum_data, lambda);
 }
+SHM_HD Float light_sampler_inv_n(const SceneView& sv) { return sv.inv_n_lights != 0.0f ? sv.inv_n_lights : 1.0f / (Float)sv.n_lights; }
 SHM_HD int light_sampler_sample(const SceneView& sv, Float u, Float& p) {
     if (sv.n_lights == 0) return -1;
     uint32_t idx = (uint32_t)(u * (Float)sv.n_lights);
     if (idx > sv.n_lights - 1) idx = sv.n_lights - 1;
-    p = 1.0f / (Float)sv.n_lights;
+    p = light_sampler_inv_n(sv);
     return (int)idx;
 }
-SHM_HD Float light_sampler_pmf(const SceneView& sv) { return sv.n_lights == 0 ? 0.0f : 1.0f / (Float)sv.n_lights; }
+SHM_HD Float light_sampler_pmf(const SceneView& sv) { return sv.n_lights == 0 ? 0.0f : light_sampler_inv_n(sv); }
 
 template <bool HAS_TEX = false>
 SHM_HD BSDF get_bsdf(const SceneView& sv, SurfaceInteraction& si, const ShmMaterial& m_in, Wavelengths& lambda, const Differentials* df = nullptr) {
diff --git a/shimmer_amd/csrc/shm/sampling.h b/shimmer_amd/csrc/shm/sampling.h
--- a/shimmer_amd/csrc/shm/sampling.h
+++ b/shimmer_amd/csrc/shm/sampling.h
@@ -367,7 +367,30 @@
     return abs(2.0f * atan2(dot(a, cross(b, c)), 1.0f + dot(a, b) + dot(a, c) + dot(b, c)));
 }
 
-SHM_HD Float sample_spherical_triangle(const V3 v[3], V3 p, V2 u, Float b[3], bool strict = false) {
+struct alignas(16) TriSampleRec {
+    V3 e1, e2;
+    V3 n;
+    Float e1e1;
+    Float inv_e1e1;
+    Float area;
+    Float inv_area;
+    Float pad[3];
+};
+static_assert(sizeof(TriSampleRec) == 64, "TriSampleRec is one 64-byte slot");
+SHM_HD TriSampleRec tri_sample_rec(V3 p0, V3 p1, V3 p2) {
+    TriSampleRec r;
+    r.e1 = p1 - p0;
+    r.e2 = p2 - p0;
+    r.n = normalize(cross(r.e1, r.e2));
+    r.e1e1 = dot(r.e1, r.e1);
+    r.inv_e1e1 = 1.0f / r.e1e1;
+    r.area = 0.5f * length(cross(r.e1, r.e2));
+    r.inv_area = 1.0f / r.area;
+    r.pad[0] = r.pad[1] = r.pad[2] = 0.0f;
+    return r;
+}
+
+SHM_HD Float sample_spherical_triangle(const V3 v[3], const TriSampleRec& rc, V3 p, V2 u, Float b[3], bool strict = false) {
     V3 a = v[0] - p, bb = v[1] - p, c = v[2] - p;
     a = normalize(a);
     bb = normalize(bb);
@@ -407,15 +430,15 @@
     Float sin_theta = safe_sqrt(1.0f - cos_theta * cos_theta);
     V3 w = cos_theta * bb + sin_theta * normalize(gram_schmidt(cp, bb));
 
-    V3 e1 = v[1] - v[0];
-    V3 e2 = v[2] - v[0];
+    V3 e1 = rc.e1;
+    V3 e2 = rc.e2;
     V3 s1 = cross(w, e2);
-    Float divisor = strict ? dot(s1, e1) : dot(e1, e1);
+    Float divisor = strict ? dot(s1, e1) : rc.e1e1;
     if (divisor == 0.0f) {
         b[0] = b[1] = b[2] = 1.0f / 3.0f;
         return pdf;
     }
-    Float inv_divisor = 1.0f / divisor;
+    Float inv_divisor = strict ? 1.0f / divisor : rc.inv_e1e1;
     V3 s = p - v[0];
     Float b1 = dot(s, s1) * inv_divisor;
     Float b2 = dot(w, cross(s, e1)) * inv_divisor;
@@ -438,6 +461,10 @@
     return pdf;
 }
 
+SHM_HD Float sample_spherical_triangle(const V3 v[3], V3 p, V2 u, Float b[3], bool strict = false) {
+    return sample_spherical_triangle(v, tri_sample_rec(v[0], v[1], v[2]), p, u, b, strict);
+}
+
 SHM_HD V2 invert_spherical_triangle_sample(const V3 v[3], V3 p, V3 w) {
     V3 a = normalize(v[0] - p), b = normalize(v[1] - p), c = normalize(v[2] - p);
     V3 n_ab = cross(a, b), n_bc = cross(b, c), n_ca = cross(c, a);
diff --git a/shimmer_amd/csrc/shm/scene.h b/shimmer_amd/csrc/shm/scene.h
--- a/shimmer_amd/csrc/shm/scene.h
+++ b/shimmer_amd/csrc/shm/scene.h
@@ -30,6 +30,12 @@
 constexpr uint32_t PRIM_SPHERE_BIT = 0x80000000u;
 
 enum : uint32_t { MESH_HAS_N = 1, MESH_HAS_S = 2, MESH_HAS_UV = 4, MESH_FLIP = 8 };
+
+union LightSampleRec {
+    TriSampleRec tri;
+    PatchSampleRec patch;
+};
+static_assert(sizeof(LightSampleRec) == 128 && alignof(LightSampleRec) == 16, "LightSampleRec is two 16-byte aligned 64-byte slots");
 
 struct SceneView {
     const ShmBvhNode* nodes;
@@ -86,6 +92,8 @@
     const SceneView* call_copy;
     const ShmBvhNode* inst_roots;
     const struct TriShadeRec* tri_shade;
+    const LightSampleRec* light_sample_recs;
+    Float inv_n_lights;
 };
 
 constexpr int FTEX_MAX_OPS = 32;
@@ -179,6 +187,24 @@
 
 SHM_HD PatchData load_patch(const SceneView& sv, uint32_t slot) { return load_patch_rec(sv, sv.prim_recs[slot]); }
 
+SHM_HD LightSampleRec light_sample_rec_of(const SceneView& sv, const ShmLight& light) {
+    LightSampleRec r;
+    r.patch = PatchSampleRec{};
+    if (light.kind != SHM_LIGHT_DIFFUSE_AREA) return r;
+    const PrimRec& pr = sv.prim_recs[light.primitive];
+    if (pr.kind_index & PRIM_SPHERE_BIT) return r;
+    if (pr.kind_index & PRIM_PATCH_BIT) r.patch = patch_sample_rec(ld3(pr.p0), ld3(pr.p1), ld3(pr.p2), ld3(sv.patches[pr.kind_index & PRIM_INDEX_MASK].p11));
+    else r.tri = tri_sample_rec(ld3(pr.p0), ld3(pr.p1), ld3(pr.p2));
+    return r;
+}
+SHM_HD const LightSampleRec* light_sample_rec(const SceneView& sv, const ShmLight& light) {
+#if defined(SHM_LIGHT_SAMPLE_RECS) && SHM_LIGHT_SAMPLE_RECS
+    return sv.light_sample_recs + (&light - sv.lights);
+#else
+    return sv.light_sample_recs ? sv.light_sample_recs + (&light - sv.lights) : nullptr;
+#endif
+}
+
 struct Hit {
     int32_t prim;
     Float t;
diff --git a/shimmer_amd/csrc/shm/shapes.h b/shimmer_amd/csrc/shm/shapes.h
--- a/shimmer_amd/csrc/shm/shapes.h
+++ b/shimmer_amd/csrc/shm/shapes.h
@@ -502,15 +502,16 @@
     Float pdf;
 };
 
-SHM_HD Float triangle_area(const TriangleData& tr) { return 0.5f * length(cross(tr.p1 - tr.p0, tr.p2 - tr.p0)); }
+SHM_HD TriSampleRec tri_sample_rec(const TriangleData& tr) { return tri_sample_rec(tr.p0, tr.p1, tr.p2); }
+SHM_HD Float triangle_area(const TriangleData& tr) { return tri_sample_rec(tr).area; }
 SHM_HD Float triangle_solid_angle(const TriangleData& tr, V3 p) {
     return spherical_triangle_area(normalize(tr.p0 - p), normalize(tr.p1 - p), normalize(tr.p2 - p));
 }
-SHM_HD ShapeSample triangle_sample(const TriangleData& tr, V2 u, bool strict = false) {
+SHM_HD ShapeSample triangle_sample(const TriangleData& tr, const TriSampleRec& rc, V2 u, bool strict = false) {
     Float b0, b1, b2;
     sample_uniform_triangle(u, b0, b1, b2);
     V3 p = b0 * tr.p0 + b1 * tr.p1 + b2 * tr.p2;
-    V3 n = normalize(cross(tr.p1 - tr.p0, tr.p2 - tr.p0));
+    V3 n = rc.n;
     if (!tr.has_n) {
         if (!strict || tr.flip) n = n * -1.0f;
     } else {
@@ -522,15 +523,16 @@
     ShapeSample ss;
     ss.pi = p3i_from_value_and_error(p, p_error);
     ss.n = n;
-    ss.pdf = 1.0f / triangle_area(tr);
+    ss.pdf = rc.inv_area;
     return ss;
 }
+SHM_HD ShapeSample triangle_sample(const TriangleData& tr, V2 u, bool strict = false) { return triangle_sample(tr, tri_sample_rec(tr), u, strict); }
 constexpr Float MIN_SPHERICAL_SAMPLE_AREA = 3e-4f;
 constexpr Float MAX_SPHERICAL_SAMPLE_AREA = 6.22f;
-SHM_HD bool triangle_sample_with_context(const TriangleData& tr, const ShapeSampleContext& ctx, V2 u, ShapeSample& out, bool strict = false) {
+SHM_HD bool triangle_sample_with_context(const TriangleData& tr, const TriSampleRec& rc, const ShapeSampleContext& ctx, V2 u, ShapeSample& out, bool strict = false) {
     Float solid_angle = triangle_solid_angle(tr, ctx.p());
     if (solid_angle < MIN_SPHERICAL_SAMPLE_AREA || solid_angle > MAX_SPHERICAL_SAMPLE_AREA) {
-        ShapeSample ss = triangle_sample(tr, u, strict);
+        ShapeSample ss = triangle_sample(tr, rc, u, strict);
         V3 wi = ss.pi.mid() - ctx.p();
         if (length_squared(wi) == 0.0f) return false;
         wi = normalize(wi);
@@ -551,13 +553,13 @@
     }
     V3 verts[3] = {tr.p0, tr.p1, tr.p2};
     Float b[3];
-    Float tri_pdf = sample_spherical_triangle(verts, ctx.p(), u, b, strict);
+    Float tri_pdf = sample_spherical_triangle(verts, rc, ctx.p(), u, b, strict);
     if (tri_pdf == 0.0f) return false;
     pdf = pdf * tri_pdf;
     V3 p_abs_sum = abs3(b[0] * tr.p0) + abs3(b[1] * tr.p1) + abs3((1.0f - b[0] - b[1]) * tr.p2);
     V3 p_error = gamma(6) * p_abs_sum;
     V3 p = b[0] * tr.p0 + b[1] * tr.p1 + b[2] * tr.p2;
-    V3 n = normalize(cross(tr.p1 - tr.p0, tr.p2 - tr.p0));
+    V3 n = rc.n;
     if (tr.has_n) {
         V3 ns = b[0] * tr.n0 + b[1] * tr.n1 + b[2] * tr.n2;
         n = face_forward(n, ns);
@@ -569,14 +571,17 @@
     out.pdf = pdf;
     return true;
 }
-SHM_HD Float triangle_pdf_with_context(const TriangleData& tr, const ShapeSampleContext& ctx, V3 wi) {
+SHM_HD bool triangle_sample_with_context(const TriangleData& tr, const ShapeSampleContext& ctx, V2 u, ShapeSample& out, bool strict = false) {
+    return triangle_sample_with_context(tr, tri_sample_rec(tr), ctx, u, out, strict);
+}
+SHM_HD Float triangle_pdf_with_context(const TriangleData& tr, const TriSampleRec& rc, const ShapeSampleContext& ctx, V3 wi) {
     Float solid_angle = triangle_solid_angle(tr, ctx.p());
     if (solid_angle < MIN_SPHERICAL_SAMPLE_AREA || solid_angle > MAX_SPHERICAL_SAMPLE_AREA) {
         V3 o = offset_ray_origin(ctx.pi, ctx.n, wi);
         TriangleIntersection ti;
         if (!intersect_triangle(o, wi, infinity(), tr.p0, tr.p1, tr.p2, ti)) return 0.0f;
         SurfaceInteraction isect = triangle_interaction(tr, ti, -wi);
-        Float pdf = (1.0f / triangle_area(tr)) / (abs_dot(isect.n, -wi) / distance_squared(ctx.p(), isect.p()));
+        Float pdf = rc.inv_area / (abs_dot(isect.n, -wi) / distance_squared(ctx.p(), isect.p()));
         if (is_inf(pdf)) return 0.0f;
         return pdf;
     }
@@ -591,6 +596,9 @@
         pdf *= bilinear_pdf(u, w);
     }
     return pdf;
+}
+SHM_HD Float triangle_pdf_with_context(const TriangleData& tr, const ShapeSampleContext& ctx, V3 wi) {
+    return triangle_pdf_with_context(tr, tri_sample_rec(tr), ctx, wi);
 }
 
 SHM_HD Float sphere_area(const ShmSphere& s) { return s.phi_max * s.radius * (s.z_max - s.z_min); }
diff --git a/shimmer_amd/csrc/wavefront.h b/shimmer_amd/csrc/wavefront.h
--- a/shimmer_amd/csrc/wavefront.h
+++ b/shimmer_amd/csrc/wavefront.h
@@ -21,6 +21,7 @@
 #define K_SPHERICAL_CAMERA false
 #endif
 #define SHM_SPHERICAL_CAMERA K_SPHERICAL_CAMERA
+#define SHM_LIGHT_SAMPLE_RECS 1
 #include "shm/path.h"
 #include "shm/tri_shade.h"
 #define WF_CAT_(a, b) a##b
@@ -167,7 +168,9 @@
 
 constexpr uint32_t LDS_TABLE_BUDGET = 12 * 1024, LDS_TABLE_BUDGET_SMALL = 1536;
 enum : int { LT_MESH_FLAGS, LT_LIGHTS, LT_LIGHT_PRIMS, LT_MATERIALS, LT_SPECTRUM, LT_RGB2SPEC_SCALE, LT_IMAGE_TEXTURES, LT_IMAGE_LEVELS, LT_FLOAT_TEXTURES, LT_FTEX_RANGES, LT_FTEX_OPS, LT_SPECTRUM_TEXTURES,
-              LT_STEX_RANGES, LT_STEX_OPS, LT_EWA_LUT, N_LDS_TABLES };
+              LT_STEX_RANGES, LT_STEX_OPS, LT_EWA_LUT,
+              LT_LIGHT_SAMPLE_RECS,
+              N_LDS_TABLES };
 struct LdsTables {
     uint32_t bytes[N_LDS_TABLES];
 };
@@ -201,6 +204,7 @@
     SHM_STAGE_TABLE(LT_STEX_RANGES, stex_ranges, FloatTexRange)
     SHM_STAGE_TABLE(LT_STEX_OPS, stex_ops, FloatTexOp)
     SHM_STAGE_TABLE(LT_EWA_LUT, ewa_lut, Float)
+    SHM_STAGE_TABLE(LT_LIGHT_SAMPLE_RECS, light_sample_recs, LightSampleRec)
 #undef SHM_STAGE_TABLE
     __syncthreads();
     return out;
```

New measurement: 5158, median of 6. About the same (+0.4%).
